# aliabdelkader/FusionTransformer

Measured on AMD Instinct MI355X. Metric: frames/sec fwd+bwd (SemanticKITTI synth), whole job, higher is better.
Workload: dtype f32

## Files before the change

fusiontransformer_amd/_lib.py:

```python
from __future__ import annotations

import ctypes as C
import os

import torch

_HERE = os.path.dirname(os.path.abspath(__file__))
LIB_PATH = os.path.join(_HERE, "csrc", "libftx.so")

_i32, _i64, _f32, _vp, _sz = C.c_int32, C.c_int64, C.c_float, C.c_void_p, C.c_size_t

SIGNATURES = {
    "ftx_version": (C.c_int, []),
    "ftx_last_error": (C.c_char_p, []),
    "ftx_stream_scratch_bytes": (_sz, []),
    "ftx_stream_scratch_attach": (C.c_int, [_vp, _vp, _sz]),
    "ftx_stream_scratch_reset": (C.c_int, [_vp]),
    "ftx_stream_scratch_release": (C.c_int, [_vp]),
    "ftx_hash": (C.c_int, [_vp, _i64, _vp, _vp]),
    "ftx_hash_kernel": (C.c_int, [_vp, _i64, _vp, _i32, _vp, _vp]),
    "ftx_floor_coords": (C.c_int, [_vp, _i64, _i32, _vp, _vp]),
    "ftx_hashtable_capacity": (_i64, [_i64]),
    "ftx_hashtable_build": (C.c_int, [_vp, _i64, _vp, _vp, _i64, _vp]),
    "ftx_hashtable_query": (C.c_int, [_vp, _i64, _vp, _vp, _i64, _vp, _vp]),
    "ftx_count": (C.c_int, [_vp, _i64, _vp, _i64, _vp]),
    "ftx_unique_workspace_bytes": (_sz, [_i64]),
    "ftx_unique_sorted": (C.c_int, [_vp, _i64, _vp, _vp, _vp, _vp, _sz, _vp]),
    "ftx_rotate_points": (C.c_int, [_vp, _i64, _vp, _vp, _vp]),
    "ftx_sorted_rank": (C.c_int, [_vp, _vp, _i64, _vp, _i64, _vp, _vp]),
    "ftx_downsample_coords": (C.c_int, [_vp, _i64, _i32, _vp, _vp]),
    "ftx_gather_coords": (C.c_int, [_vp, _vp, _i64, _vp, _vp]),
    "ftx_levels_workspace_bytes": (_sz, [_i64, _i32]),
    "ftx_levels_unique": (C.c_int, [_vp, _i64, _vp, _i32, _vp, _vp, _vp, _vp, _vp, _vp, _sz, _vp]),
    "ftx_level_segments": (C.c_int, [_vp, _i64, _vp, _i64, _i32, _vp, _vp]),
    "ftx_level_coords": (C.c_int, [_vp, _vp, _i64, _i32, _vp, _vp]),
    "ftx_kernel_map_build": (C.c_int, [_vp, _i64, _vp, _i32, _vp, _vp, _i64, _vp, _vp]),
    "ftx_kernel_map_count_workspace_bytes": (_sz, [_i64, _i32]),
    "ftx_kernel_map_count": (C.c_int, [_vp, _i64, _i32, _vp, _vp, _vp, _sz, _vp]),
    "ftx_kernel_map_pairs": (C.c_int, [_vp, _i64, _i64, _i32, _vp, _vp, _vp, _vp, _i64, _vp]),
    "ftx_trilinear_weights": (C.c_int, [_vp, _vp, _i64, _i32, _vp, _vp]),
    "ftx_voxelize_fwd": (C.c_int, [_vp, _vp, _vp, _i64, _i32, _i64, _vp, _vp]),
    "ftx_voxelize_bwd": (C.c_int, [_vp, _vp, _vp, _i64, _i32, _i64, _vp, _vp]),
    "ftx_devoxelize_fwd": (C.c_int, [_vp, _vp, _vp, _i64, _i32, _i64, _vp, _vp]),
    "ftx_devoxelize_bwd": (C.c_int, [_vp, _vp, _vp, _i64, _i32, _i64, _vp, _vp]),
    "ftx_segment_workspace_bytes": (_sz, [_i64, _i64]),
    "ftx_segment_build": (C.c_int, [_vp, _i64, _i64, _vp, _vp, _vp, _sz, _vp]),
    "ftx_voxelize_fwd_sorted": (C.c_int, [_vp, _vp, _vp, _i64, _i32, _i64, _vp, _vp]),
    "ftx_devoxelize_bwd_sorted": (C.c_int, [_vp, _vp, _vp, _vp, _i64, _i32, _i64, _vp, _vp]),
    "ftx_segment_sum": (C.c_int, [_vp, _vp, _vp, _i64, _i32, _i64, _vp, _vp]),
    "ftx_lift_cells": (C.c_int, [_vp, _vp, _i64, _i32, _i32, _i32, _i32, _i32, _vp, _vp]),
    "ftx_lift_gather_fwd": (C.c_int, [_vp, _vp, _vp, _i64, _i32, _i32, _i32, _i32, _i32, _i32, _vp, _vp]),
    "ftx_lift_gather_bwd": (C.c_int, [_vp, _vp, _vp, _i64, _i32, _i32, _i32, _i32, _i32, _i32, _vp, _vp]),
    "ftx_resample_nearest_fwd": (C.c_int, [_vp, _i32, _i32, _i32, _i32, _i32, _i32, _vp, _vp]),
    "ftx_resample_nearest_bwd": (C.c_int, [_vp, _i32, _i32, _i32, _i32, _i32, _i32, _vp, _vp]),
    "ftx_sample_down_workspace_bytes": (_sz, []),
    "ftx_sample_down_fwd": (C.c_int, [_vp, _i32, _i32, _i32, _i32, _i32, _vp, _vp, _vp, _vp, _vp, _vp, _f32, _f32, _i32, _vp, _vp, _vp, _sz, _vp]),
    "ftx_sample_down_bwd": (C.c_int, [_vp, _vp, _i32, _i32, _i32, _i32, _i32, _vp, _vp, _vp, _vp, _vp, _vp, _vp, _vp, _vp, _sz, _vp]),
    "ftx_affine_sample_fwd": (C.c_int, [_vp, _vp, _i32, _i32, _i32, _i32, _vp, _i32, _i32, _vp, _vp]),
    "ftx_affine_theta_workspace_bytes": (_sz, [_i32]),
    "ftx_affine_sample_bwd_theta": (C.c_int, [_vp, _vp, _i32, _i32, _i32, _i32, _vp, _vp, _i32, _i32, _vp, _vp, _sz, _vp]),
    "ftx_affine_lift_fwd": (C.c_int, [_vp, _vp, _i32, _i32, _i32, _i32, _vp, _vp, _vp, _i64, _i32, _i32, _vp, _vp]),
    "ftx_affine_lift_cells": (C.c_int, [_vp, _vp, _vp, _i64, _i32, _i32, _i32, _i32, _i32, _vp, _vp]),
    "ftx_affine_lift_bwd": (C.c_int, [_vp, _vp, _i32, _i32, _i32, _i32, _vp, _vp, _vp, _vp, _i64, _i32, _i32, _vp, _vp, _vp, _vp, _vp, _sz, _vp]),
    "ftx_loc_conv_pool_relu_fwd_workspace_bytes": (_sz, [_i32, _i32, _i32, _i32]),
    "ftx_loc_conv_pool_relu_fwd": (C.c_int, [_vp, _vp, _i32, _i32, _i32, _i32, _vp, _vp, _i32, _i32, _vp, _vp, _vp, _vp, _sz, _vp]),
    "ftx_loc_conv_pool_relu_bwd_weight_workspace_bytes": (_sz, [_i32, _i32, _i32, _i32, _i32, _i32]),
    "ftx_loc_conv_pool_relu_bwd_weight": (C.c_int, [_vp, _vp, _i32, _i32, _i32, _i32, _vp, _vp, _vp, _i32, _i32, _vp, _vp, _vp, _sz, _vp]),
    "ftx_loc_conv_pool_relu_bwd_data": (C.c_int, [_vp, _vp, _vp, _vp, _i32, _i32, _i32, _i32, _i32, _i32, _vp, _vp, _vp]),
    "ftx_spconv_pairs_gemm": (C.c_int, [_vp, _i64, _vp, _vp, _i32, _vp, _i64, _i32, _i32, _i32, _vp, _vp]),
    "ftx_spconv_pairs_gemm_scatter": (C.c_int, [_vp, _i64, _vp, _vp, _vp, _i32, _vp, _i64, _i32, _i32, _i32, _vp, _i64, _vp]),
    "ftx_spconv_ostat_supported": (_i32, [_i32, _i32, _i32, _i32]),
    "ftx_spconv_ostat_blocks": (_i32, [_i64]),
    "ftx_spconv_ostat": (C.c_int, [_vp, _i64, _vp, _i64, _vp, _i32, _i32, _i32, _i32, _i32, _vp, _vp, _i32, _vp]),
    "ftx_rows_gemm": (C.c_int, [_vp, _i64, _vp, _i32, _vp, _i32, _i32, _vp, _vp]),
    "ftx_spconv_gemm_block_cols": (_i32, [_i32, _i64, _i32]),
    "ftx_spconv_reduce": (C.c_int, [_vp, _vp, _i64, _i32, _i32, _vp, _vp]),
    "ftx_spconv_reduce_bn_eval": (C.c_int, [_vp, _vp, _i64, _i32, _i32, _vp, _vp, _vp, _vp, _vp, _f32, _i32, _vp, _vp]),
    "ftx_spconv_reduce_stats_blocks": (_i32, [_i64, _i32]),
    "ftx_spconv_reduce_stats": (C.c_int, [_vp, _vp, _i64, _i32, _i32, _vp, _vp, _i32, _vp]),
    "ftx_bn_train_fwd_totals": (C.c_int, [_vp, _vp, _vp, _vp, _vp, _vp, _f32, _f32, _i64, _i32, _i32, _vp, _vp, _vp, _vp, _vp]),
    "ftx_spconv_pairs_wgrad_workspace_bytes": (_sz, [_i64, _i32, _i32, _i32]),
    "ftx_spconv_pairs_wgrad": (C.c_int, [_vp, _i64, _vp, _vp, _i64, _vp, _vp, _i64, _i32, _i32, _i32, _vp, _vp, _sz, _vp]),
    "ftx_spconv_wgrad_resident_blocks": (_i32, [_i32, _i32]),
    "ftx_spconv_wgrad_table_blocks": (_i32, [_i32, _i32, _i32, _i32]),
    "ftx_spconv_pairs_gemm_bf16": (C.c_int, [_vp, _i64, _vp, _vp, _i32, _vp, _i64, _i32, _i32, _i32, _vp, _vp]),
    "ftx_spconv_pairs_gemm_scatter_bf16": (C.c_int, [_vp, _i64, _vp, _vp, _vp, _i32, _vp, _i64, _i32, _i32, _i32, _vp, _i64, _vp]),
    "ftx_rows_gemm_bf16": (C.c_int, [_vp, _i64, _vp, _i32, _vp, _i32, _i32, _vp, _vp]),
    "ftx_spconv_pairs_wgrad_bf16_workspace_bytes": (_sz, [_i64, _i32, _i32, _i32]),
    "ftx_spconv_pairs_wgrad_bf16": (C.c_int, [_vp, _i64, _vp, _vp, _i64, _vp, _vp, _i64, _i32, _i32, _i32, _vp, _vp, _sz, _vp]),
    "ftx_spconv_gemm_bf16_block_cols": (_i32, [_i32, _i64, _i32]),
    "ftx_spconv_wgrad_bf16_table_blocks": (_i32, [_i32, _i32, _i32, _i32]),
    "ftx_bn_workspace_bytes": (_sz, [_i64, _i32]),
    "ftx_bn_train_fwd": (C.c_int, [_vp, _vp, _vp, _vp, _vp, _vp, _f32, _f32, _i64, _i32, _i32, _vp, _vp, _vp, _vp, _sz, _vp]),
    "ftx_bn_eval_fwd": (C.c_int, [_vp, _vp, _vp, _vp, _vp, _vp, _f32, _i64, _i32, _i32, _vp, _vp]),
    "ftx_adam_chunk_elements": (_i32, []),
    "ftx_adam_tensor_bytes": (_i32, []),
    "ftx_adam_step": (C.c_int, [_vp, _vp, _vp, _i32, C.c_double, C.c_double, _f32, _f32, _vp]),
    "ftx_add_layernorm_fwd": (C.c_int, [_vp, _vp, _vp, _vp, _vp, _f32, _i64, _i32, _vp, _vp, _vp, _vp, _vp]),
    "ftx_layernorm_bwd_workspace_bytes": (_sz, [_i64, _i32]),
    "ftx_add_layernorm_bwd": (C.c_int, [_vp, _vp, _vp, _vp, _vp, _vp, _i64, _i32, _i32, _vp, _vp, _vp, _sz, _vp]),
    "ftx_colsum_workspace_bytes": (_sz, [_i64, _i32]),
    "ftx_colsum": (C.c_int, [_vp, _i64, _i32, _vp, _vp, _sz, _vp]),
    "ftx_attn_fwd": (C.c_int, [_vp, _i32, _i32, _i32, _i32, _f32, _vp, _vp, _vp]),
    "ftx_attn_bwd_workspace_bytes": (_sz, [_i32, _i32, _i32]),
    "ftx_attn_bwd": (C.c_int, [_vp, _vp, _vp, _vp, _i32, _i32, _i32, _i32, _f32, _vp, _vp, _sz, _vp]),
    "ftx_attn_fwd_tiled": (C.c_int, [_vp, _i32, _i32, _i32, _i32, _f32, _vp, _vp, _i32, _i32, _vp]),
    "ftx_attn_bwd_tiled": (C.c_int, [_vp, _vp, _vp, _vp, _i32, _i32, _i32, _i32, _f32, _vp, _vp, _sz, _i32, _i32, _vp]),
    "ftx_attn_fwd_bf16": (C.c_int, [_vp, _i32, _i32, _i32, _i32, _f32, _vp, _vp, _i32, _i32, _vp]),
    "ftx_attn_bwd_bf16": (C.c_int, [_vp, _vp, _vp, _vp, _i32, _i32, _i32, _i32, _f32, _vp, _vp, _sz, _i32, _i32, _vp]),
    "ftx_dense_gemm_bf16": (C.c_int, [_vp, _vp, _i32, _vp, _vp, _i64, _i32, _i32, _i32, _vp, _vp, _vp]),
    "ftx_dense_wgrad_bf16_workspace_bytes": (_sz, [_i64, _i32, _i32]),
    "ftx_dense_wgrad_bf16": (C.c_int, [_vp, _vp, _i64, _i32, _i32, _vp, _vp, _sz, _vp]),
    "ftx_dense_bf16_tile": (C.c_int, [_i32, _i64, _i32, _i32, _vp, _vp, _vp]),
    "ftx_dense_gemm_split": (C.c_int, [_vp, _vp, _i32, _vp, _vp, _i64, _i32, _i32, _i32, _vp, _vp, _vp]),
    "ftx_dense_wgrad_split_workspace_bytes": (_sz, [_i64, _i32, _i32]),
    "ftx_dense_wgrad_split": (C.c_int, [_vp, _vp, _i64, _i32, _i32, _vp, _vp, _sz, _vp]),
    "ftx_dense_split_tile": (C.c_int, [_i32, _i64, _i32, _i32, _vp, _vp, _vp]),
    "ftx_fusion_loss_workspace_bytes": (_sz, []),
    "ftx_fusion_loss": (C.c_int, [_vp, _vp, _vp, _vp, _vp, _vp, _f32, _i64, _i32, _i32, _vp, _vp, _vp, _vp, _vp, _vp, _vp, _vp, _sz, _vp]),
    "ftx_fusion_loss_mix": (C.c_int, [_vp, _vp, _vp, _vp, _vp, _vp, _f32, _f32, _i64, _i32, _i32, _vp, _vp, _vp, _vp, _vp, _vp, _vp, _vp, _sz, _vp]),
    "ftx_seg_loss_workspace_bytes": (_sz, []),
    "ftx_seg_loss": (C.c_int, [_vp, _vp, _vp, _i64, _i32, _i32, _vp, _vp, _vp, _vp, _sz, _vp]),
    "ftx_project_points": (C.c_int, [_vp, _i64, _vp, _i32, _i32, _vp, _vp, _vp]),
    "ftx_eval_scatter_back": (C.c_int, [_vp, _vp, _i64, _i32, _vp, _vp, _i64, _vp, _vp, _vp, _vp, _vp, _vp, _vp, _vp, _vp]),
    "ftx_bn_train_bwd": (C.c_int, [_vp, _vp, _vp, _vp, _vp, _vp, _vp, _i64, _i32, _i32, _vp, _vp, _vp, _vp, _vp, _sz, _vp]),
    "ftx_color_jitter_workspace_bytes": (_sz, [_i32, _i32]),
    "ftx_color_jitter_u8": (C.c_int, [_vp, _i64, _i32, _i32, _i32, _vp, _vp, _i32, _vp, _vp, _sz, _vp]),
    "ftx_color_jitter_chw": (C.c_int, [_vp, _i64, _i32, _i32, _i32, _vp, _vp, _i32, _i32, _vp, _vp, _vp, _vp, _sz, _vp]),
    "ftx_resize_ksize": (_i32, [_i32, _i32]),
    "ftx_resize_coeffs_host": (C.c_int, [_i32, _i32, _vp, _vp]),
    "ftx_resize_workspace_bytes": (_sz, [_i32, _i32, _i32, _i32, _i32]),
    "ftx_resize_bilinear_u8": (C.c_int, [_vp, _i64, _i64, _i32, _i32, _i32, _i32, _vp, _vp, _i32, _vp, _vp, _i32, _i32, _i32, _vp, _vp, _sz, _vp]),
    "ftx_rows_concat": (C.c_int, [_vp, _i32, _vp, _i32, _i64, _vp, _vp]),
    "ftx_rows_add": (C.c_int, [_vp, _vp, _i64, _i32, _vp, _vp]),
    "ftx_spvcnn_layer_bytes": (_i32, []),
    "ftx_spvcnn_op_bytes": (_i32, []),
    "ftx_spvcnn_map_bytes": (_i32, []),
    "ftx_spvcnn_pv_bytes": (_i32, []),
    "ftx_spvcnn_eval_arena_bytes": (_sz, [_vp, _i32, _vp, _i32, _vp, _vp, _i32, _vp, _i32, _vp]),
    "ftx_spvcnn_eval": (C.c_int, [_vp, _i32, _vp, _i32, _vp, _vp, _i32, _vp, _i32, _vp, _vp, _i32, _i32, _vp, _vp, _vp, _sz, _vp, _vp]),
    "ftx_rows_split": (C.c_int, [_vp, _i64, _i32, _i32, _vp, _vp, _vp]),
    "ftx_spvcnn_train_layer_bytes": (_i32, []),
    "ftx_spvcnn_train_pv_bytes": (_i32, []),
    "ftx_spvcnn_train_arena_bytes": (_sz, [_vp, _i32, _vp, _i32, _vp, _vp, _i32, _vp, _i32, _vp, _vp]),
    "ftx_spvcnn_train_fwd": (C.c_int, [_vp, _vp, _i32, _vp, _i32, _vp, _vp, _i32, _vp, _i32, _vp, _vp, _i32, _i32, _vp, _vp, _vp, _vp, _sz, _vp, _vp, _vp]),
    "ftx_spvcnn_train_bwd": (C.c_int, [_vp, _vp, _i32, _vp, _i32, _vp, _vp, _i32, _vp, _vp, _i32, _vp, _vp, _i32, _i32, _vp, _vp, _vp, _sz, _vp, _vp]),
    "ftx_spvcnn_index_layout_words": (_i32, []),
    "ftx_spvcnn_index_layout": (C.c_int, [_i64, _i32, _vp, _vp, _i32, _vp]),
    "ftx_spvcnn_index_levels_arena_bytes": (_sz, [_i64]),
    "ftx_spvcnn_index_maps_arena_bytes": (_sz, [_i64, _i32, _vp, _i32]),
    "ftx_spvcnn_index_pairs_arena_bytes": (_sz, [_i64, _vp, _vp]),
    "ftx_spvcnn_index_levels": (C.c_int, [_vp, _i64, _f32, _f32, _vp, _sz, _vp, _vp]),
    "ftx_spvcnn_index_maps": (C.c_int, [_vp, _i64, _f32, _f32, _vp, _i32, _vp, _i32, _vp, _sz, _vp, _sz, _vp, _vp]),
# ... 60 lines not shown
```

fusiontransformer_amd/csrc/ftx_spconv.hip:

```cpp
#include <cstring>
#include <cstdlib>
#include "ftx_bn_eval_op.h"
#include "ftx_index_ops.h"
#include "ftx_spconv_common.h"
#include <rocprim/device/device_scan.hpp>
#include <rocprim/iterator/transform_iterator.hpp>

using namespace ftx;

struct IsValid {
  __host__ __device__ int32_t operator()(int32_t v) const { return v >= 0 ? 1 : 0; }
};

extern "C" size_t ftx_kernel_map_count_workspace_bytes(int64_t n_out, int32_t k) {
  if (n_out <= 0 || k <= 0) return 256;
  size_t bytes = 0;
  const int32_t *in = nullptr;
  int32_t *out = nullptr;
  auto it = rocprim::make_transform_iterator(in, IsValid());
  if (rocprim::exclusive_scan(nullptr, bytes, it, out, 0, (size_t)(n_out * k), rocprim::plus<int32_t>()) != hipSuccess) return 0;
  return bytes + 256;
}

__global__ void koff_kernel(const int32_t *__restrict__ nbr, const int32_t *__restrict__ scan, int64_t n_out, int k, int32_t *__restrict__ koff) {
  int t = blockIdx.x * blockDim.x + threadIdx.x;
  if (t <= k) koff[t] = koff_entry(nbr, scan, n_out, k, t, 0);
}

extern "C" int ftx_kernel_map_count(const int32_t *nbr, int64_t n_out, int32_t k, int32_t *pos, int32_t *koff, void *workspace,
                                    size_t workspace_bytes, void *stream) {
  FTX_REQUIRE(n_out >= 0 && k >= 1, "ftx_kernel_map_count: bad size");
  FTX_REQUIRE(koff, "ftx_kernel_map_count: null koff");
  hipStream_t st = (hipStream_t)stream;
  if (n_out == 0) {
    if (hipMemsetAsync(koff, 0, sizeof(int32_t) * (k + 1), st) != hipSuccess) return check_launch("ftx_kernel_map_count memset");
    return FTX_OK;
  }
  FTX_REQUIRE(nbr && pos && workspace, "ftx_kernel_map_count: null pointer");
  FTX_REQUIRE(n_out * k < 0x7fffffff, "ftx_kernel_map_count: map too large for int32 positions");
  size_t need = ftx_kernel_map_count_workspace_bytes(n_out, k);
  if (workspace_bytes < need) return workspace_short("ftx_kernel_map_count", workspace_bytes, need);
  size_t bytes = workspace_bytes;
  auto it = rocprim::make_transform_iterator(nbr, IsValid());
  if (rocprim::exclusive_scan(workspace, bytes, it, pos, 0, (size_t)(n_out * k), rocprim::plus<int32_t>(), st) != hipSuccess) {
    set_error("ftx_kernel_map_count: scan failed");
    return FTX_ELAUNCH;
  }
  koff_kernel<<<1, 64, 0, st>>>(nbr, pos, n_out, k, koff);
  return check_launch("ftx_kernel_map_count");
}

__global__ void fill_m1_kernel(int32_t *__restrict__ p, int64_t n) {
  for (int64_t i = blockIdx.x * (int64_t)blockDim.x + threadIdx.x; i < n; i += (int64_t)gridDim.x * blockDim.x) p[i] = -1;
}

__global__ void pairs_scatter_kernel(const int32_t *__restrict__ nbr, int64_t n_out, int64_t n_in, int k, int32_t *__restrict__ pos,
                                     int32_t *__restrict__ pos_t, int32_t *__restrict__ pair_in, int32_t *__restrict__ pair_out,
                                     int64_t cap) {
  const int64_t total = n_out * k;
  for (int64_t e = blockIdx.x * (int64_t)blockDim.x + threadIdx.x; e < total; e += (int64_t)gridDim.x * blockDim.x) {
    if (pair_entry(nbr[e], pos[e], e, n_out, n_in, cap, pair_in, pair_out, pos_t) < 0) pos[e] = -1;
  }
}

extern "C" int ftx_kernel_map_pairs(const int32_t *nbr, int64_t n_out, int64_t n_in, int32_t k, int32_t *pos, int32_t *pos_t, int32_t *pair_in,
                                    int32_t *pair_out, int64_t n_pairs, void *stream) {
  FTX_REQUIRE(n_out >= 0 && n_in >= 0 && k >= 1 && n_pairs >= 0, "ftx_kernel_map_pairs: bad size");
  hipStream_t st = (hipStream_t)stream;
  if (n_in > 0) {
    FTX_REQUIRE(pos_t, "ftx_kernel_map_pairs: null pos_t");
    fill_m1_kernel<<<grid_for(n_in * k, 256), 256, 0, st>>>(pos_t, n_in * k);
  }
  if (n_out == 0) return check_launch("ftx_kernel_map_pairs");
  FTX_REQUIRE(nbr && pos && (n_pairs == 0 || (pair_in && pair_out)), "ftx_kernel_map_pairs: null pointer");
  pairs_scatter_kernel<<<grid_for(n_out * k, 256), 256, 0, st>>>(nbr, n_out, n_in, k, pos, pos_t, pair_in, pair_out, n_pairs);
  return check_launch("ftx_kernel_map_pairs");
}

constexpr int AS_STRIDE = 36;

template <int NT>
__global__ __launch_bounds__(256) void pairs_gemm_kernel(const float *__restrict__ A, int64_t rows_a, const int32_t *__restrict__ gather,
                                                         const float *__restrict__ W, int w_transposed, const int32_t *__restrict__ koff,
                                                         int ca, int co, int kvol, float *__restrict__ tmp, const float *__restrict__ bias,
                                                         int64_t n_dense, const int32_t *__restrict__ scatter, int64_t rows_out) {
  constexpr int BN = 32 * NT;
  constexpr int BS_STRIDE = AS_STRIDE;
  constexpr int A_PASSES = kPairAPasses;
  constexpr int B_PASSES = NT;

  __shared__ __attribute__((aligned(16))) float As[kPairTile * AS_STRIDE];
  __shared__ __attribute__((aligned(16))) float Bs[BN * BS_STRIDE];
  __shared__ int s_tile[3];

  const int tid = threadIdx.x;
  gemm_tile_scan(koff, kvol, n_dense, gather == nullptr, s_tile);
  __syncthreads();
  const int k = s_tile[0];
  if (k < 0) return;
  const int p0 = s_tile[1], cnt = s_tile[2];

  const int wave = tid >> 6, lane = tid & 63;
  const int half = lane >> 5, l31 = lane & 31;
  const int n0 = blockIdx.y * BN;
  const int arow = tid >> 3, acol = (tid & 7) * 4;

  const bool kfull = (ca % kPairBK) == 0;
  int32_t src[A_PASSES];
  pair_gather_rows(gather, p0, cnt, rows_a, src);
  const float *Wk = W + (int64_t)k * ca * co;

  f32x16 acc[NT];
#pragma unroll
  for (int j = 0; j < NT; ++j)
#pragma unroll
    for (int g = 0; g < 16; ++g) acc[j][g] = 0.f;

  float4 ra[A_PASSES], rb[B_PASSES];
  auto load_chunk = [&](int c0) {
    if (kfull) {
#pragma unroll
      for (int p = 0; p < A_PASSES; ++p) ra[p] = *(const float4 *)&A[(int64_t)src[p] * ca + c0 + acol];
#pragma unroll
      for (int q = 0; q < B_PASSES; ++q) {
        if (!w_transposed) {
          int kk = ((tid >> 6) << 3) + (tid & 7), n4 = n0 + (q * 8 + ((tid >> 3) & 7)) * 4;
          n4 = n4 + 4 <= co ? n4 : co - 4;
          rb[q] = *(const float4 *)&Wk[(int64_t)(c0 + kk) * co + n4];
        } else {
          int e = q * 256 + tid;
          int nn = n0 + (e >> 3), k4 = (e & 7) * 4;
          nn = nn < co ? nn : co - 1;
          rb[q] = *(const float4 *)&Wk[(int64_t)nn * ca + c0 + k4];
        }
      }
      return;
    }
#pragma unroll
    for (int p = 0; p < A_PASSES; ++p) {
      float4 v = make_float4(0.f, 0.f, 0.f, 0.f);
      if (c0 + acol < ca) v = *(const float4 *)&A[(int64_t)src[p] * ca + c0 + acol];
      ra[p] = v;
    }
#pragma unroll
    for (int q = 0; q < B_PASSES; ++q) {
      float4 v = make_float4(0.f, 0.f, 0.f, 0.f);
      if (!w_transposed) {
        int kk = ((tid >> 6) << 3) + (tid & 7), n4 = (q * 8 + ((tid >> 3) & 7)) * 4;
        if (c0 + kk < ca && n0 + n4 < co) v = *(const float4 *)&Wk[(int64_t)(c0 + kk) * co + n0 + n4];
      } else {
        int e = q * 256 + tid;
        int nn = e >> 3, k4 = (e & 7) * 4;
        if (n0 + nn < co && c0 + k4 < ca) v = *(const float4 *)&Wk[(int64_t)(n0 + nn) * ca + c0 + k4];
      }
      rb[q] = v;
    }
  };
  auto store_chunk = [&]() {
#pragma unroll
    for (int p = 0; p < A_PASSES; ++p) *(float4 *)&As[(p * 32 + arow) * AS_STRIDE + acol] = ra[p];
#pragma unroll
    for (int q = 0; q < B_PASSES; ++q) {
      if (!w_transposed) {
        int kk = ((tid >> 6) << 3) + (tid & 7), n4 = (q * 8 + ((tid >> 3) & 7)) * 4;
        Bs[(n4 + 0) * BS_STRIDE + kk] = rb[q].x;
        Bs[(n4 + 1) * BS_STRIDE + kk] = rb[q].y;
        Bs[(n4 + 2) * BS_STRIDE + kk] = rb[q].z;
        Bs[(n4 + 3) * BS_STRIDE + kk] = rb[q].w;
      } else {
        int e = q * 256 + tid;
        int nn = e >> 3, k4 = (e & 7) * 4;
        *(float4 *)&Bs[nn * BS_STRIDE + k4] = rb[q];
      }
    }
  };

  load_chunk(0);
  for (int c0 = 0; c0 < ca; c0 += kPairBK) {
    store_chunk();
    __syncthreads();
    if (c0 + kPairBK < ca) load_chunk(c0 + kPairBK);
    const float *arow_p = &As[(wave * 32 + l31) * AS_STRIDE + 4 * half];
    const float *brow_p = &Bs[l31 * BS_STRIDE + 4 * half];
    float af[2][4], bf[2][NT][4];
    auto load_frag = [&](int buf, int t) {
      float4 a = *(const float4 *)(arow_p + 8 * t);
      af[buf][0] = a.x; af[buf][1] = a.y; af[buf][2] = a.z; af[buf][3] = a.w;
#pragma unroll
      for (int j = 0; j < NT; ++j) {
        float4 b = *(const float4 *)(brow_p + j * 32 * BS_STRIDE + 8 * t);
        bf[buf][j][0] = b.x; bf[buf][j][1] = b.y; bf[buf][j][2] = b.z; bf[buf][j][3] = b.w;
      }
    };
    load_frag(0, 0);
#pragma unroll
    for (int t = 0; t < kPairBK / 8; ++t) {
      if (t + 1 < kPairBK / 8) load_frag((t + 1) & 1, t + 1);
#pragma unroll
      for (int s = 0; s < 4; ++s)
#pragma unroll
        for (int j = 0; j < NT; ++j) acc[j] = __builtin_amdgcn_mfma_f32_32x32x2f32(bf[t & 1][j][s], af[t & 1][s], acc[j], 0, 0, 0);
    }
    __syncthreads();
  }
  pair_gemm_epilogue<NT>(acc, p0, cnt, n0, gather, rows_a, scatter, rows_out, bias, co, tmp);
}

#include "ftx_lastblock.h"


template <int KVOL>
__device__ __forceinline__ float4 reduce_row(const float *__restrict__ tmp, const int32_t *__restrict__ pos, int64_t n, int co, int kvol,
                                             int64_t r, int j) {
  float4 acc = make_float4(0.f, 0.f, 0.f, 0.f);
  if (KVOL > 0) {
    int32_t p[KVOL > 0 ? KVOL : 1];
#pragma unroll
    for (int k = 0; k < KVOL; ++k) p[k] = pos[(int64_t)k * n + r];
#pragma unroll
    for (int k = 0; k < KVOL; ++k) {
      if (p[k] >= 0) {
        float4 v = *(const float4 *)&tmp[(int64_t)p[k] * co + j];
        acc.x += v.x; acc.y += v.y; acc.z += v.z; acc.w += v.w;
      }
    }
  } else {
    for (int k = 0; k < kvol; ++k) {
      int32_t q = pos[(int64_t)k * n + r];
      if (q >= 0) {
        float4 v = *(const float4 *)&tmp[(int64_t)q * co + j];
        acc.x += v.x; acc.y += v.y; acc.z += v.z; acc.w += v.w;
      }
    }
  }
  return acc;
}

template <int KVOL>
__global__ void spconv_reduce_kernel(const float *__restrict__ tmp, const int32_t *__restrict__ pos, int64_t n, int co, int kvol,
                                     float *__restrict__ out) {
  const int cv = co >> 2;
  const int64_t total = n * cv;
  for (int64_t e = blockIdx.x * (int64_t)blockDim.x + threadIdx.x; e < total; e += (int64_t)gridDim.x * blockDim.x) {
    int64_t r = e / cv;
    int j = (int)(e - r * cv) * 4;
    const float4 acc = reduce_row<KVOL>(tmp, pos, n, co, kvol, r, j);
    *(float4 *)&out[r * co + j] = acc;
  }
}

static unsigned reduce_grid(int64_t n, int co) {
  int64_t g = ceil_div(n * (co / 4), 256);
  if (g > 8192) g = 8192;
  return (unsigned)g;
}

extern "C" int ftx_spconv_reduce(const float *tmp, const int32_t *pos, int64_t n, int32_t co, int32_t kvol, float *out, void *stream) {
  FTX_REQUIRE(n >= 0 && kvol >= 1 && co >= 4 && co % 4 == 0, "ftx_spconv_reduce: bad size");
  if (n == 0) return FTX_OK;
  FTX_REQUIRE(pos && out, "ftx_spconv_reduce: null pointer");
  const unsigned g = reduce_grid(n, co);
  hipStream_t st = (hipStream_t)stream;
  if (kvol == 27)
    spconv_reduce_kernel<27><<<g, 256, 0, st>>>(tmp, pos, n, co, kvol, out);
  else if (kvol == 8)
    spconv_reduce_kernel<8><<<g, 256, 0, st>>>(tmp, pos, n, co, kvol, out);
  else
    spconv_reduce_kernel<0><<<g, 256, 0, st>>>(tmp, pos, n, co, kvol, out);
  return check_launch("ftx_spconv_reduce");
}

template <int KVOL>
__global__ void spconv_reduce_bn_eval_kernel(const float *__restrict__ tmp, const int32_t *__restrict__ pos, int64_t n, int co,
                                             const float *__restrict__ res, const float *__restrict__ gamma, const float *__restrict__ beta,
                                             const float *__restrict__ rm, const float *__restrict__ rv, float eps, int relu,
                                             float *__restrict__ out) {
  const int cv = co >> 2;
  const int64_t total = n * cv;
  for (int64_t e = blockIdx.x * (int64_t)blockDim.x + threadIdx.x; e < total; e += (int64_t)gridDim.x * blockDim.x) {
    int64_t r = e / cv;
    int j = (int)(e - r * cv) * 4;
    const float4 acc = reduce_row<KVOL>(tmp, pos, n, co, KVOL, r, j);
    *(float4 *)&out[r * co + j] = bn_eval_apply4(acc, res, r * co + j, rm, rv, eps, gamma, beta, j, relu);
  }
}

extern "C" int ftx_spconv_reduce_bn_eval(const float *tmp, const int32_t *pos, int64_t n, int32_t co, int32_t kvol, const float *residual,
                                         const float *gamma, const float *beta, const float *running_mean, const float *running_var,
// ... 149 lines not shown
        if (p >= rend || s_ok[(p - rbase) & (kWgradRound - 1)] == 0) rg[q] = make_float4(0.f, 0.f, 0.f, 0.f);
      }
    }
#pragma unroll
    for (int q = 0; q < QA; ++q) *(float4 *)&As[(q * 256 + tid) * 4] = ra[q];
#pragma unroll
    for (int q = 0; q < QG; ++q) *(float4 *)&Gs[(q * 256 + tid) * 4] = rg[q];
  };
  const float *ap = As + wm * 32 * MI + MI * l31, *gp = Gs + wn * 32 * NI + NI * l31;
  auto mfma_step = [&]() {
    constexpr int ITS = WG_BR / 2 / KS;
    float af[2][MI], gf[2][NI];
    auto frag = [&](int buf, int it) {
      const int kk = 2 * (it * KS + ks) + half;
      FragLoad<MI>::ld(ap + kk * TM, af[buf]);
      FragLoad<NI>::ld(gp + kk * TN, gf[buf]);
    };
    frag(0, 0);
#pragma unroll
    for (int it = 0; it < ITS; ++it) {
      if (it + 1 < ITS) frag((it + 1) & 1, it + 1);
#pragma unroll
      for (int i = 0; i < MI; ++i)
#pragma unroll
        for (int j = 0; j < NI; ++j)
          acc[i][j] = __builtin_amdgcn_mfma_f32_32x32x2f32(gf[it & 1][j], af[it & 1][i], acc[i][j], 0, 0, 0);
    }
  };

  for (rbase = lo; rbase < hi; rbase += kWgradRound) {
    rend = (rbase + kWgradRound < hi) ? rbase + kWgradRound : hi;
    wgrad_stage_indices(idx_a, rows_a, idx_g, rows_g, rbase, rend, s_ia, s_ig, s_ok, &s_bad);
    load_step(rbase, ra0, rg0);
    load_step(rbase + WG_BR, ra1, rg1);
    for (int p0 = rbase; p0 < rend; p0 += 2 * WG_BR) {
      store_step(p0, ra0, rg0);
      __syncthreads();
      load_step(p0 + 2 * WG_BR, ra0, rg0);
      mfma_step();
      __syncthreads();
      if (p0 + WG_BR >= rend) break;
      store_step(p0 + WG_BR, ra1, rg1);
      __syncthreads();
      load_step(p0 + 3 * WG_BR, ra1, rg1);
      mfma_step();
      __syncthreads();
    }
  }

  wgrad_ks_reduce<MI, NI, KS>(acc, lds, wq, ks, lane);

  if (ks == 0) {
    const int64_t mat = (int64_t)ca * cg;
    float *dst = single ? dW + (int64_t)k * mat : part + (int64_t)blockIdx.x * mat;
    const int ab = m0 + wm * 32 * MI + MI * l31, gb = n0 + wn * 32 * NI;
#pragma unroll
    for (int i = 0; i < MI; ++i) {
      const int row = ab + i;
      if (row < ca) {
#pragma unroll
        for (int q = 0; q < 4; ++q) {
          float v[4 * NI];
#pragma unroll
          for (int e = 0; e < 4; ++e)
#pragma unroll
            for (int j = 0; j < NI; ++j) v[e * NI + j] = acc[i][j][4 * q + e];
          const int col = gb + NI * (8 * q + 4 * half);
#pragma unroll
          for (int t = 0; t < NI; ++t)
            if (col + 4 * t < cg) *(float4 *)&dst[(int64_t)row * cg + col + 4 * t] = make_float4(v[4 * t], v[4 * t + 1], v[4 * t + 2], v[4 * t + 3]);
        }
      }
    }
  }
}

struct SpconvF32 {
  static constexpr const char *pairs_name = "ftx_spconv_pairs_gemm", *scatter_name = "ftx_spconv_pairs_gemm_scatter", *rows_name = "ftx_rows_gemm",
                              *wgrad_name = "ftx_spconv_pairs_wgrad";
  static constexpr int wgrad_blocks[4][4] = {{8, 4, 3, 3}, {5, 3, 2, 2}, {4, 2, 1, 2}, {3, 2, 2, 2}};
  static constexpr int wgrad_step = 2 * WG_BR;
  template <int NT>
  static void gemm(dim3 grid, hipStream_t st, const PairsGemmArgs &a) {
    pairs_gemm_kernel<NT><<<grid, 256, 0, st>>>(a.A, a.rows_a, a.gather, a.W, a.w_transposed, a.koff, a.ca, a.co, a.kvol, a.out, a.bias, a.n_dense,
                                                a.scatter, a.rows_out);
  }
  template <int MI, int NI, int WMG, int WNG>
  static void wgrad(dim3 grid, hipStream_t st, const PairsWgradArgs &a) {
    pairs_wgrad_kernel<MI, NI, WMG, WNG><<<grid, 256, 0, st>>>(a.A, a.rows_a, a.idx_a, a.G, a.rows_g, a.idx_g, a.koff, a.ca, a.cg, a.kvol, a.tile_len,
                                                               a.part, a.dW, a.n_dense);
  }
};

extern "C" int32_t ftx_spconv_gemm_block_cols(int32_t co, int64_t n_pairs, int32_t kvol) { return spconv_gemm_block_cols(co, n_pairs, kvol); }

extern "C" int ftx_spconv_pairs_gemm(const float *A, int64_t rows_a, const int32_t *gather, const float *W, int32_t w_transposed,
                                     const int32_t *koff, int64_t n_pairs, int32_t ca, int32_t co, int32_t kvol, float *tmp, void *stream) {
  return spconv_pairs_entry<SpconvF32>(false, A, rows_a, gather, nullptr, W, w_transposed, koff, n_pairs, ca, co, kvol, tmp, 0, stream);
}

extern "C" int ftx_spconv_pairs_gemm_scatter(const float *A, int64_t rows_a, const int32_t *gather, const int32_t *scatter, const float *W,
                                             int32_t w_transposed, const int32_t *koff, int64_t n_pairs, int32_t ca, int32_t co, int32_t kvol,
                                             float *out, int64_t rows_out, void *stream) {
  return spconv_pairs_entry<SpconvF32>(true, A, rows_a, gather, scatter, W, w_transposed, koff, n_pairs, ca, co, kvol, out, rows_out, stream);
}

extern "C" int ftx_rows_gemm(const float *A, int64_t n, const float *W, int32_t w_transposed, const float *bias, int32_t ca, int32_t co,
                             float *out, void *stream) {
  return spconv_rows_entry<SpconvF32>(A, n, W, w_transposed, bias, ca, co, out, stream);
}

extern "C" int32_t ftx_spconv_wgrad_table_blocks(int32_t mi, int32_t wmg, int32_t ni, int32_t wng) {
  return spconv_wgrad_table_blocks<SpconvF32>(mi, wmg, ni, wng);
}
extern "C" int32_t ftx_spconv_wgrad_resident_blocks(int32_t ca, int32_t cg) { return spconv_wgrad_occ<SpconvF32>(spconv_wgrad_config(ca, cg)); }

extern "C" size_t ftx_spconv_pairs_wgrad_workspace_bytes(int64_t n_pairs, int32_t ca, int32_t cg, int32_t kvol) {
  return spconv_wgrad_workspace_bytes<SpconvF32>(n_pairs, ca, cg, kvol);
}

extern "C" int ftx_spconv_pairs_wgrad(const float *A, int64_t rows_a, const int32_t *idx_a, const float *G, int64_t rows_g, const int32_t *idx_g,
                                      const int32_t *koff, int64_t n_pairs, int32_t ca, int32_t cg, int32_t kvol, float *dW, void *workspace,
                                      size_t workspace_bytes, void *stream) {
  return spconv_wgrad_entry<SpconvF32>(A, rows_a, idx_a, G, rows_g, idx_g, koff, n_pairs, ca, cg, kvol, dW, workspace, workspace_bytes, stream);
}
```

fusiontransformer_amd/csrc/ftx_spconv_bf16.hip:

```cpp
#include "ftx_spconv_common.h"

using namespace ftx;

__device__ inline bf16x4 round4(float4 v) { return (bf16x4){(__bf16)v.x, (__bf16)v.y, (__bf16)v.z, (__bf16)v.w}; }

constexpr int GB_STRIDE = 40;

template <int NT>
__global__ __launch_bounds__(256) void pairs_gemm_bf16_kernel(const float *__restrict__ A, int64_t rows_a, const int32_t *__restrict__ gather,
                                                              const float *__restrict__ W, int w_transposed, const int32_t *__restrict__ koff,
                                                              int ca, int co, int kvol, float *__restrict__ tmp, const float *__restrict__ bias,
                                                              int64_t n_dense, const int32_t *__restrict__ scatter, int64_t rows_out) {
  constexpr int BN = 32 * NT;
  constexpr int A_PASSES = kPairAPasses;
  constexpr int B_PASSES = NT;
  __shared__ __attribute__((aligned(16))) __bf16 As[kPairTile * GB_STRIDE];
  __shared__ __attribute__((aligned(16))) __bf16 Bs[BN * GB_STRIDE];
  __shared__ int s_tile[3];

  const int tid = threadIdx.x;
  gemm_tile_scan(koff, kvol, n_dense, gather == nullptr, s_tile);
  __syncthreads();
  const int k = s_tile[0];
  if (k < 0) return;
// ... 188 lines not shown
      for (int e = 0; e < 4; ++e) *(bf16x2 *)&At[(ra_row[q] + e) * WB_STRIDE + pa[q]] = (bf16x2){x0[e], x1[e]};
    }
#pragma unroll
    for (int q = 0; q < QG; ++q) {
      const bf16x4 x0 = round4(rg[q][0]), x1 = round4(rg[q][1]);
#pragma unroll
      for (int e = 0; e < 4; ++e) *(bf16x2 *)&Gt[(rg_row[q] + e) * WB_STRIDE + pg[q]] = (bf16x2){x0[e], x1[e]};
    }
  };
  const __bf16 *ap = At + (wm * MI * 32 + l31) * WB_STRIDE + 8 * half;
  const __bf16 *gp = Gt + (wn * NI * 32 + l31) * WB_STRIDE + 8 * half;
  auto mfma_step = [&]() {
#pragma unroll
    for (int it = 0; it < 4 / KS; ++it) {
      const int s = it * KS + ks;
      bf16x8 af[MI], gf[NI];
#pragma unroll
      for (int i = 0; i < MI; ++i) af[i] = *(const bf16x8 *)(ap + i * 32 * WB_STRIDE + 16 * s);
#pragma unroll
      for (int j = 0; j < NI; ++j) gf[j] = *(const bf16x8 *)(gp + j * 32 * WB_STRIDE + 16 * s);
#pragma unroll
      for (int i = 0; i < MI; ++i)
#pragma unroll
        for (int j = 0; j < NI; ++j) acc[i][j] = mfma_bf16(gf[j], af[i], acc[i][j]);
    }
  };

  for (rbase = lo; rbase < hi; rbase += kWgradRound) {
    rend = (rbase + kWgradRound < hi) ? rbase + kWgradRound : hi;
    wgrad_stage_indices(idx_a, rows_a, idx_g, rows_g, rbase, rend, s_ia, s_ig, s_ok, &s_bad);
    load_step(rbase);
    for (int p0 = rbase; p0 < rend; p0 += WB_BR) {
      store_step(p0);
      __syncthreads();
      if (p0 + WB_BR < rend) load_step(p0 + WB_BR);
      mfma_step();
      __syncthreads();
    }
  }

  wgrad_ks_reduce<MI, NI, KS>(acc, (float *)lds, wq, ks, lane);

  if (ks == 0) {
    const int64_t mat = (int64_t)ca * cg;
    float *dst = single ? dW + (int64_t)k * mat : part + (int64_t)blockIdx.x * mat;
#pragma unroll
    for (int i = 0; i < MI; ++i) {
      const int row = m0 + (wm * MI + i) * 32 + l31;
      if (row < ca) {
#pragma unroll
        for (int j = 0; j < NI; ++j)
#pragma unroll
          for (int q = 0; q < 4; ++q) {
            const int col = n0 + (wn * NI + j) * 32 + 8 * q + 4 * half;
            if (col < cg)
              *(float4 *)&dst[(int64_t)row * cg + col] = make_float4(acc[i][j][4 * q], acc[i][j][4 * q + 1], acc[i][j][4 * q + 2], acc[i][j][4 * q + 3]);
          }
      }
    }
  }
}

struct SpconvBf16 {
  static constexpr const char *pairs_name = "ftx_spconv_pairs_gemm_bf16", *scatter_name = "ftx_spconv_pairs_gemm_scatter_bf16",
                              *rows_name = "ftx_rows_gemm_bf16", *wgrad_name = "ftx_spconv_pairs_wgrad_bf16";
  static constexpr int wgrad_blocks[4][4] = {{8, 4, 3, 3}, {4, 3, 2, 2}, {3, 2, 1, 2}, {3, 2, 2, 2}};
  static constexpr int wgrad_step = 2 * WB_BR;
  template <int NT>
  static void gemm(dim3 grid, hipStream_t st, const PairsGemmArgs &a) {
    pairs_gemm_bf16_kernel<NT><<<grid, 256, 0, st>>>(a.A, a.rows_a, a.gather, a.W, a.w_transposed, a.koff, a.ca, a.co, a.kvol, a.out, a.bias, a.n_dense,
                                                     a.scatter, a.rows_out);
  }
  template <int MI, int NI, int WMG, int WNG>
  static void wgrad(dim3 grid, hipStream_t st, const PairsWgradArgs &a) {
    pairs_wgrad_bf16_kernel<MI, NI, WMG, WNG><<<grid, 256, 0, st>>>(a.A, a.rows_a, a.idx_a, a.G, a.rows_g, a.idx_g, a.koff, a.ca, a.cg, a.kvol,
                                                                    a.tile_len, a.part, a.dW, a.n_dense);
  }
};

extern "C" int32_t ftx_spconv_gemm_bf16_block_cols(int32_t co, int64_t n_pairs, int32_t kvol) { return spconv_gemm_block_cols(co, n_pairs, kvol); }

extern "C" int ftx_spconv_pairs_gemm_bf16(const float *A, int64_t rows_a, const int32_t *gather, const float *W, int32_t w_transposed,
                                          const int32_t *koff, int64_t n_pairs, int32_t ca, int32_t co, int32_t kvol, float *tmp, void *stream) {
  return spconv_pairs_entry<SpconvBf16>(false, A, rows_a, gather, nullptr, W, w_transposed, koff, n_pairs, ca, co, kvol, tmp, 0, stream);
}

extern "C" int ftx_spconv_pairs_gemm_scatter_bf16(const float *A, int64_t rows_a, const int32_t *gather, const int32_t *scatter, const float *W,
                                                  int32_t w_transposed, const int32_t *koff, int64_t n_pairs, int32_t ca, int32_t co, int32_t kvol,
                                                  float *out, int64_t rows_out, void *stream) {
  return spconv_pairs_entry<SpconvBf16>(true, A, rows_a, gather, scatter, W, w_transposed, koff, n_pairs, ca, co, kvol, out, rows_out, stream);
}

extern "C" int ftx_rows_gemm_bf16(const float *A, int64_t n, const float *W, int32_t w_transposed, const float *bias, int32_t ca, int32_t co,
                                  float *out, void *stream) {
  return spconv_rows_entry<SpconvBf16>(A, n, W, w_transposed, bias, ca, co, out, stream);
}

extern "C" int32_t ftx_spconv_wgrad_bf16_table_blocks(int32_t mi, int32_t wmg, int32_t ni, int32_t wng) {
  return spconv_wgrad_table_blocks<SpconvBf16>(mi, wmg, ni, wng);
}

extern "C" size_t ftx_spconv_pairs_wgrad_bf16_workspace_bytes(int64_t n_pairs, int32_t ca, int32_t cg, int32_t kvol) {
  return spconv_wgrad_workspace_bytes<SpconvBf16>(n_pairs, ca, cg, kvol);
}

extern "C" int ftx_spconv_pairs_wgrad_bf16(const float *A, int64_t rows_a, const int32_t *idx_a, const float *G, int64_t rows_g, const int32_t *idx_g,
                                           const int32_t *koff, int64_t n_pairs, int32_t ca, int32_t cg, int32_t kvol, float *dW, void *workspace,
                                           size_t workspace_bytes, void *stream) {
  return spconv_wgrad_entry<SpconvBf16>(A, rows_a, idx_a, G, rows_g, idx_g, koff, n_pairs, ca, cg, kvol, dW, workspace, workspace_bytes, stream);
}
```

fusiontransformer_amd/csrc/ftx_spconv_common.h:

```cpp
#pragma once
#include "ftx_common.h"
#include "ftx_mfma.h"

namespace ftx {

constexpr int kPairTile = 128;
constexpr int kPairBK = 32;
constexpr int kPairAPasses = 4;
constexpr int kWgradRound = 1024;
constexpr int kWgradCUs = 256;

template <bool RANGE>
__device__ __forceinline__ void pair_tile_scan(const int32_t *__restrict__ koff, int kvol, int tile, int n_dense, int *s_tile) {
  const int tid = threadIdx.x, b = blockIdx.x;
  if (tid >= 64) return;
  int c = 0;
  if (tid < kvol) c = koff ? koff[tid + 1] - koff[tid] : n_dense;
  int nt = (c + tile - 1) / tile;
  int incl = nt;
#pragma unroll
  for (int off = 1; off < 64; off <<= 1) {
    int v = __shfl_up(incl, off, 64);
    if (tid >= off) incl += v;
  }
  int excl = incl - nt;
  bool mine = (tid < kvol) && b >= excl && b < incl;
  unsigned long long m = __ballot(mine);
  if (mine) {
    int t = b - excl;
    int left = c - t * tile;
    int first = (koff ? koff[tid] : 0) + t * tile;
    s_tile[0] = tid;
    s_tile[1] = first;
    s_tile[2] = (RANGE ? first : 0) + (left > tile ? tile : left);
    if (RANGE) s_tile[3] = nt;
  }
  if (m == 0ull && tid == 0) s_tile[0] = -1;
}

__device__ __forceinline__ void gemm_tile_scan(const int32_t *__restrict__ koff, int kvol, int64_t n_dense, bool dense, int *s_tile) {
  if (!dense) {
    __builtin_assume(koff != nullptr);
    return pair_tile_scan<false>(koff, kvol, kPairTile, 0, s_tile);
  }
  if (threadIdx.x == 0) {
    int64_t left = n_dense - (int64_t)blockIdx.x * kPairTile;
    s_tile[0] = left > 0 ? 0 : -1;
    s_tile[1] = blockIdx.x * kPairTile;
    s_tile[2] = left > kPairTile ? kPairTile : (int)left;
  }
}

__device__ __forceinline__ void pair_gather_rows(const int32_t *__restrict__ gather, int p0, int cnt, int64_t rows_a, int32_t (&src)[kPairAPasses]) {
  const int arow = threadIdx.x >> 3;
#pragma unroll
  for (int p = 0; p < kPairAPasses; ++p) {
    int r = p * 32 + arow;
    int32_t s = 0;
    if (r < cnt) s = gather ? gather[p0 + r] : p0 + r;
    if (s < 0 || s >= rows_a) s = 0;
    src[p] = s;
  }
}

template <int NT>
__device__ __forceinline__ void pair_gemm_epilogue(const f32x16 (&acc)[NT], int p0, int cnt, int n0, const int32_t *__restrict__ gather, int64_t rows_a,
                                          const int32_t *__restrict__ scatter, int64_t rows_out, const float *__restrict__ bias, int co,
                                          float *__restrict__ out) {
  const int wave = threadIdx.x >> 6, lane = threadIdx.x & 63;
  const int half = lane >> 5, l31 = lane & 31;
  const bool nfull = n0 + 32 * NT <= co;
  const int row = wave * 32 + l31;
  int64_t drow = row < cnt ? p0 + row : -1;
  bool zero = false;
  if (gather != nullptr && drow >= 0) {
    const int32_t sidx = gather[drow];
    zero = sidx < 0 || sidx >= rows_a;
  }
  if (scatter != nullptr && drow >= 0) {
    drow = scatter[drow];
    if (drow >= rows_out) drow = -1;
  }
  if (drow < 0) return;
  float *dst = out + drow * co;
#pragma unroll
  for (int j = 0; j < NT; ++j)
#pragma unroll
    for (int q = 0; q < 4; ++q) {
      const int col = n0 + j * 32 + 8 * q + 4 * half;
      if (nfull || col < co) {
        float4 v = make_float4(acc[j][4 * q], acc[j][4 * q + 1], acc[j][4 * q + 2], acc[j][4 * q + 3]);
        if (zero) v = make_float4(0.f, 0.f, 0.f, 0.f);
        if (bias) {
          const float4 bv = *(const float4 *)&bias[col];
          v.x += bv.x; v.y += bv.y; v.z += bv.z; v.w += bv.w;
        }
        *(float4 *)&dst[col] = v;
      }
    }
}

__device__ __forceinline__ void wgrad_stage_indices(const int32_t *__restrict__ idx_a, int64_t rows_a, const int32_t *__restrict__ idx_g, int64_t rows_g,
                                           int rbase, int rend, int32_t *s_ia, int32_t *s_ig, uint8_t *s_ok, int *s_bad) {
  __syncthreads();
  if (threadIdx.x == 0) *s_bad = 0;
  __syncthreads();
  for (int t = threadIdx.x; t < kWgradRound; t += 256) {
    int32_t ia = 0, ig = 0;
    uint8_t ok = 0;
    if (t < rend - rbase) {
      ia = idx_a ? idx_a[rbase + t] : rbase + t;
      ig = idx_g ? idx_g[rbase + t] : rbase + t;
      ok = 1;
      if (ia < 0 || ia >= rows_a || ig < 0 || ig >= rows_g) {
        ia = ig = 0;
        ok = 0;
        *s_bad = 1;
      }
    }
    s_ia[t] = ia;
    s_ig[t] = ig;
    s_ok[t] = ok;
  }
  __syncthreads();
}

template <int MI, int NI, int KS>
__device__ __forceinline__ void wgrad_ks_reduce(f32x16 (&acc)[MI][NI], float *red, int wq, int ks, int lane) {
  for (int r = 1; r < KS; ++r) {
    if (ks == r) {
#pragma unroll
      for (int i = 0; i < MI; ++i)
#pragma unroll
        for (int j = 0; j < NI; ++j) {
          const f32x16 v = acc[i][j];
#pragma unroll
          for (int g = 0; g < 16; ++g) red[(((wq * MI + i) * NI + j) * 16 + g) * 64 + lane] = v[g];
        }
    }
    __syncthreads();
    if (ks == 0) {
#pragma unroll
      for (int i = 0; i < MI; ++i)
#pragma unroll
        for (int j = 0; j < NI; ++j) {
          f32x16 v = acc[i][j];
#pragma unroll
          for (int g = 0; g < 16; ++g) v[g] += red[(((wq * MI + i) * NI + j) * 16 + g) * 64 + lane];
          acc[i][j] = v;
        }
    }
    __syncthreads();
  }
}

}

template <int TL>
__global__ __launch_bounds__(256) void wgrad_reduce_kernel(const float *__restrict__ part, const int32_t *__restrict__ koff, int kvol,
                                                           int tile_len, int n_dense, int64_t mat, float *__restrict__ dW) {
  constexpr int COLS = 256 / TL;
  __shared__ float4 sh[TL][COLS];
  const int k = blockIdx.y;
  int first = 0, cnt = 0;
  for (int q = 0; q <= k; ++q) {
    int c = koff ? koff[q + 1] - koff[q] : n_dense;
    int nt = (c + tile_len - 1) / tile_len;
    if (q < k) first += nt; else cnt = nt;
  }
  if (cnt == 1) return;
  const int col = threadIdx.x % COLS, tl = threadIdx.x / COLS;
  const int64_t chunks = ftx::ceil_div(mat / 4, COLS);
  for (int64_t chunk = blockIdx.x; chunk < chunks; chunk += gridDim.x) {
    const int64_t e = (chunk * COLS + col) * 4;
    float4 s = make_float4(0.f, 0.f, 0.f, 0.f);
    if (e < mat) {
      const float *src = part + (int64_t)first * mat + e;
      int t = tl;
      for (; t + 3 * TL < cnt; t += 4 * TL) {
        float4 v0 = *(const float4 *)&src[(int64_t)t * mat], v1 = *(const float4 *)&src[(int64_t)(t + TL) * mat];
        float4 v2 = *(const float4 *)&src[(int64_t)(t + 2 * TL) * mat], v3 = *(const float4 *)&src[(int64_t)(t + 3 * TL) * mat];
        s.x += v0.x; s.y += v0.y; s.z += v0.z; s.w += v0.w;
        s.x += v1.x; s.y += v1.y; s.z += v1.z; s.w += v1.w;
        s.x += v2.x; s.y += v2.y; s.z += v2.z; s.w += v2.w;
        s.x += v3.x; s.y += v3.y; s.z += v3.z; s.w += v3.w;
      }
      for (; t < cnt; t += TL) {
        float4 v = *(const float4 *)&src[(int64_t)t * mat];
        s.x += v.x; s.y += v.y; s.z += v.z; s.w += v.w;
      }
    }
    if (TL > 1) {
      sh[tl][col] = s;
      __syncthreads();
      if (tl == 0) {
#pragma unroll
        for (int l = 1; l < TL; ++l) {
          float4 v = sh[l][col];
          s.x += v.x; s.y += v.y; s.z += v.z; s.w += v.w;
        }
      }
      __syncthreads();
    }
    if (tl == 0 && e < mat) *(float4 *)&dW[(int64_t)k * mat + e] = s;
  }
}

namespace ftx {

inline void launch_wgrad_reduce(const float *part, const int32_t *koff, int kvol, int tile_len, int n_dense, int64_t mat, int64_t tiles, float *dW,
                                hipStream_t st) {
  const int64_t big_tiles = kvol > 1 ? 6 * tiles / kvol : tiles;
  const int64_t want_blocks = ceil_div(1024, kvol);
  auto rgrid = [&](int cols) { int64_t c = ceil_div(mat / 4, cols); return dim3((unsigned)(c < want_blocks ? c : want_blocks), (unsigned)kvol); };
  if (big_tiles <= 4)
    wgrad_reduce_kernel<1><<<rgrid(256), 256, 0, st>>>(part, koff, kvol, tile_len, n_dense, mat, dW);
  else if (big_tiles <= 32)
    wgrad_reduce_kernel<4><<<rgrid(64), 256, 0, st>>>(part, koff, kvol, tile_len, n_dense, mat, dW);
  else
    wgrad_reduce_kernel<16><<<rgrid(16), 256, 0, st>>>(part, koff, kvol, tile_len, n_dense, mat, dW);
}

struct PairsGemmArgs {
  const float *A;
  int64_t rows_a;
  const int32_t *gather;
  const float *W;
  int w_transposed;
  const int32_t *koff;
  int ca, co, kvol;
  float *out;
  const float *bias;
  int64_t n_dense;
  const int32_t *scatter;
  int64_t rows_out;
};

inline int spconv_gemm_nt(int co, int64_t row_tiles) {
  int nt = co >= 128 ? 4 : (co + 31) / 32;
  if (co > 128 && co % 96 == 0 && co % 128 != 0) nt = 3;
  if (nt == 4 && row_tiles * ceil_div(co, 128) <= 400) nt = 2;
  return nt;
}

inline int32_t spconv_gemm_block_cols(int32_t co, int64_t n_pairs, int32_t kvol) {
  if (co < 4 || co % 4 != 0 || n_pairs < 0 || kvol < 0) return -1;
  return 32 * spconv_gemm_nt(co, ceil_div(n_pairs, kPairTile) + kvol);
}

template <class F>
void spconv_launch_gemm(int64_t row_tiles, hipStream_t st, const PairsGemmArgs &a) {
  const int nt = spconv_gemm_nt(a.co, row_tiles);
  const dim3 grid((unsigned)row_tiles, (unsigned)ceil_div(a.co, 32 * nt));
  switch (nt) {
    case 1: F::template gemm<1>(grid, st, a); break;
    case 2: F::template gemm<2>(grid, st, a); break;
    case 3: F::template gemm<3>(grid, st, a); break;
    default: F::template gemm<4>(grid, st, a); break;
  }
}

template <class F>
int spconv_pairs_entry(bool scattered, const float *A, int64_t rows_a, const int32_t *gather, const int32_t *scatter, const float *W,
                       int32_t w_transposed, const int32_t *koff, int64_t n_pairs, int32_t ca, int32_t co, int32_t kvol, float *out, int64_t rows_out,
                       void *stream) {
  const char *me = scattered ? F::scatter_name : F::pairs_name;
  FTX_REQUIRE(n_pairs >= 0 && rows_a >= 0 && rows_out >= 0 && kvol >= 1 && kvol <= 64, "%s: bad size", me);
  FTX_REQUIRE(ca >= 4 && ca % 4 == 0 && co >= 4 && co % 4 == 0, "%s: channels must be multiples of 4 (ca=%d co=%d)", me, ca, co);
  if (n_pairs == 0) return FTX_OK;
  FTX_REQUIRE(A && gather && (scatter || !scattered) && W && koff && out && rows_a >= 1, "%s: null pointer or empty operand", me);
  const PairsGemmArgs a = {A, rows_a, gather, W, w_transposed, koff, ca, co, kvol, out, nullptr, 0, scatter, rows_out};
  spconv_launch_gemm<F>(ceil_div(n_pairs, kPairTile) + kvol, (hipStream_t)stream, a);
  return check_launch(me);
}

template <class F>
int spconv_rows_entry(const float *A, int64_t n, const float *W, int32_t w_transposed, const float *bias, int32_t ca, int32_t co, float *out,
                      void *stream) {
  const char *me = F::rows_name;
  FTX_REQUIRE(n >= 0, "%s: n < 0", me);
  FTX_REQUIRE(ca >= 4 && ca % 4 == 0 && co >= 4 && co % 4 == 0, "%s: channels must be multiples of 4 (ca=%d co=%d)", me, ca, co);
  if (n == 0) return FTX_OK;
  FTX_REQUIRE(A && W && out, "%s: null pointer", me);
  const PairsGemmArgs a = {A, n, nullptr, W, w_transposed, nullptr, ca, co, 1, out, bias, n, nullptr, 0};
  spconv_launch_gemm<F>(ceil_div(n, kPairTile), (hipStream_t)stream, a);
  return check_launch(me);
}

struct PairsWgradArgs {
  const float *A;
  int64_t rows_a;
  const int32_t *idx_a;
  const float *G;
  int64_t rows_g;
  const int32_t *idx_g, *koff;
  int ca, cg, kvol, tile_len;
  float *part, *dW;
  int n_dense;
};

struct WgradCfg { int mi, wmg, ni, wng; };
inline WgradCfg spconv_wgrad_config(int ca, int cg) {
  WgradCfg c;
  if (ca <= 32) { c.mi = 1; c.wmg = 1; }
  else if (ca <= 64) { c.mi = 2; c.wmg = 1; }
  else if (ca % 96 == 0 && ca % 128 != 0) { c.mi = 3; c.wmg = 1; }
  else { c.mi = 2; c.wmg = 2; }
  if (cg <= 32) { c.ni = 1; c.wng = 1; }
  else if (cg <= 64) { c.ni = 2; c.wng = 1; }
  else if (cg % 96 == 0 && cg % 128 != 0) { c.ni = 3; c.wng = 1; }
  else { c.ni = 2; c.wng = 2; }
  if (c.mi == 3 && c.ni == 3) { c.mi = 2; c.wmg = 2; }
  return c;
}

template <class F>
int spconv_wgrad_occ(const WgradCfg &c) {
  auto side = [](int i, int w) { return w == 2 ? 3 : i - 1; };
  return F::wgrad_blocks[side(c.mi, c.wmg)][side(c.ni, c.wng)];
}
template <class F>
int32_t spconv_wgrad_table_blocks(int32_t mi, int32_t wmg, int32_t ni, int32_t wng) {
  if (!((mi >= 1 && mi <= 3 && wmg == 1) || (mi == 2 && wmg == 2)) || !((ni >= 1 && ni <= 3 && wng == 1) || (ni == 2 && wng == 2))) return -1;
  return spconv_wgrad_occ<F>(WgradCfg{mi, wmg, ni, wng});
}

template <class F>
int spconv_wgrad_tile_len(int64_t n_pairs, int ca, int cg, int kvol) {
  const WgradCfg c = spconv_wgrad_config(ca, cg);
  const int64_t mn_tiles = ceil_div(ca, 32 * c.mi * c.wmg) * ceil_div(cg, 32 * c.ni * c.wng);
  const int64_t slots = (int64_t)kWgradCUs * spconv_wgrad_occ<F>(c);
  int64_t len = 256;
  for (int rounds = 1; rounds <= 64; ++rounds) {
    int64_t tiles = (slots * rounds * 15 / 16) / mn_tiles - (kvol + 1) / 2;
    if (tiles < 1) tiles = 1;
    len = ceil_div(ceil_div(n_pairs, tiles), F::wgrad_step) * F::wgrad_step;
    if (len <= 4096) break;
  }
  if (len < 256) len = 256;
  return (int)len;
}

inline int64_t spconv_wgrad_tiles_ub(int64_t n_pairs, int tile_len, int kvol) { return ceil_div(n_pairs, tile_len) + kvol; }

template <class F>
size_t spconv_wgrad_workspace_bytes(int64_t n_pairs, int32_t ca, int32_t cg, int32_t kvol) {
  if (n_pairs <= 0 || ca <= 0 || cg <= 0 || kvol <= 0) return 256;
  const int len = spconv_wgrad_tile_len<F>(n_pairs, ca, cg, kvol);
  return sizeof(float) * (size_t)spconv_wgrad_tiles_ub(n_pairs, len, kvol) * ca * cg;
}

template <class F, int MI, int WMG>
void spconv_launch_wgrad_n(const WgradCfg &c, dim3 grid, hipStream_t st, const PairsWgradArgs &a) {
  if (c.ni == 1) F::template wgrad<MI, 1, WMG, 1>(grid, st, a);
  else if (c.ni == 3) F::template wgrad<MI, 3, WMG, 1>(grid, st, a);
  else if (c.wng == 1) F::template wgrad<MI, 2, WMG, 1>(grid, st, a);
  else F::template wgrad<MI, 2, WMG, 2>(grid, st, a);
}

template <class F>
int spconv_wgrad_entry(const float *A, int64_t rows_a, const int32_t *idx_a, const float *G, int64_t rows_g, const int32_t *idx_g,
                       const int32_t *koff, int64_t n_pairs, int32_t ca, int32_t cg, int32_t kvol, float *dW, void *workspace,
                       size_t workspace_bytes, void *stream) {
  const char *me = F::wgrad_name;
  FTX_REQUIRE(n_pairs >= 0 && rows_a >= 0 && rows_g >= 0 && kvol >= 1 && kvol <= 64, "%s: bad size", me);
  FTX_REQUIRE(ca >= 4 && ca % 4 == 0 && cg >= 4 && cg % 4 == 0, "%s: channels must be multiples of 4 (ca=%d cg=%d)", me, ca, cg);
  FTX_REQUIRE(dW, "%s: null dW", me);
// ... 32 lines not shown
```

fusiontransformer_amd/functional.py:

```python
from __future__ import annotations

import ctypes
import functools

import numpy as np
import torch

from . import _lib
from ._lib import check, ptr, req, stream

I32, I64, F32 = torch.int32, torch.int64, torch.float32


def _empty(shape, dtype, like):
    return torch.empty(shape, dtype=dtype, device=like.device)


_SCRATCH = {}
_WS_BYTES = {}


def _ws_bytes(fn_name, *args):
    key = (fn_name,) + args
    v = _WS_BYTES.get(key)
# ... 168 lines not shown


def sorted_rank(sorted_keys: torch.Tensor, n_sorted: torch.Tensor, queries: torch.Tensor) -> torch.Tensor:
    L = _lib.load()
    req(sorted_keys, I64, "sorted_rank sorted", 1)
    req(n_sorted, I32, "sorted_rank n_sorted", 1)
    req(queries, I64, "sorted_rank queries", 1)
    rank = _empty((queries.shape[0],), I32, queries)
    check(L.ftx_sorted_rank(ptr(sorted_keys), ptr(n_sorted), sorted_keys.shape[0], ptr(queries), queries.shape[0], ptr(rank), stream()), "ftx_sorted_rank")
    return rank


def rotate_points(points: torch.Tensor, rot) -> torch.Tensor:
    L = _lib.load()
    req(points, F32, "rotate_points points", 2)
    if points.shape[1] != 3:
        raise ValueError("rotate_points: points must be (N, 3)")
    r = np.ascontiguousarray(np.asarray(rot, dtype=np.float32).reshape(9))
    out = _empty(tuple(points.shape), F32, points)
    check(L.ftx_rotate_points(ptr(points), points.shape[0], r.ctypes.data_as(ctypes.c_void_p), ptr(out), stream()), "ftx_rotate_points")
    return out


def downsample_coords(coords: torch.Tensor, ratio: int) -> torch.Tensor:
    L = _lib.load()
    req(coords, I32, "downsample coords", 2)
    out = torch.empty_like(coords)
    check(L.ftx_downsample_coords(ptr(coords), coords.shape[0], int(ratio), ptr(out), stream()), "ftx_downsample_coords")
    return out


def gather_coords(src: torch.Tensor, index: torch.Tensor) -> torch.Tensor:
    L = _lib.load()
    req(src, I32, "gather_coords src", 2)
    req(index, I32, "gather_coords index", 1)
    out = _empty((index.shape[0], 4), I32, src)
    check(L.ftx_gather_coords(ptr(src), ptr(index), index.shape[0], ptr(out), stream()), "ftx_gather_coords")
    return out


def kernel_offsets(kernel_size: int, tensor_stride: int = 1) -> np.ndarray:
    single = (np.arange(-kernel_size // 2 + 1, kernel_size // 2 + 1) * tensor_stride).tolist()
    if kernel_size % 2 == 1:
        offs = [[x, y, z] for z in single for y in single for x in single]
    else:
        offs = [[x, y, z] for x in single for y in single for z in single]
    return np.array(offs, dtype=np.int32)


def kernel_map_build(out_coords: torch.Tensor, offsets: torch.Tensor, table: HashTable) -> torch.Tensor:
    L = _lib.load()
    req(out_coords, I32, "kernel_map out_coords", 2)
    req(offsets, I32, "kernel_map offsets", 2)
    n_out, k = out_coords.shape[0], offsets.shape[0]
    nbr = _empty((k, n_out), I32, out_coords)
    check(L.ftx_kernel_map_build(ptr(out_coords), n_out, ptr(offsets), k, ptr(table.keys), ptr(table.vals), table.capacity, ptr(nbr), stream()),
          "ftx_kernel_map_build")
    return nbr


def kernel_map_count(nbr: torch.Tensor):
    L = _lib.load()
    req(nbr, I32, "kernel_map_count nbr", 2)
    k, n_out = nbr.shape
    pos = torch.empty_like(nbr)
    koff = _empty((k + 1,), I32, nbr)
    ws_bytes = _ws_bytes("ftx_kernel_map_count_workspace_bytes", n_out, k)
    ws = _scratch(ws_bytes, nbr)
    check(L.ftx_kernel_map_count(ptr(nbr), n_out, k, ptr(pos), ptr(koff), ptr(ws), ws_bytes, stream()), "ftx_kernel_map_count")
    return pos, koff


def kernel_map_pairs(nbr: torch.Tensor, pos: torch.Tensor, n_in: int, n_pairs: int):
    L = _lib.load()
    k, n_out = nbr.shape
    pos_t = _empty((k, int(n_in)), I32, nbr)
    pair_in = _empty((int(n_pairs),), I32, nbr)
    pair_out = _empty((int(n_pairs),), I32, nbr)
    check(L.ftx_kernel_map_pairs(ptr(nbr), n_out, int(n_in), k, ptr(pos), ptr(pos_t), ptr(pair_in), ptr(pair_out), int(n_pairs), stream()),
          "ftx_kernel_map_pairs")
    return pos, pos_t, pair_in, pair_out


def calc_ti_weights(pc: torch.Tensor, idx_query: torch.Tensor, scale: int = 1) -> torch.Tensor:
    L = _lib.load()
    req(pc, F32, "calc_ti_weights pc", 2)
    req(idx_query, I32, "calc_ti_weights idx", 2)
    n = pc.shape[0]
    if pc.shape[1] != 4 or idx_query.shape != (n, 8):
        raise ValueError("calc_ti_weights: pc must be (N,4) and idx (N,8)")
    w = _empty((n, 8), F32, pc)
    check(L.ftx_trilinear_weights(ptr(pc), ptr(idx_query), n, int(scale), ptr(w), stream()), "ftx_trilinear_weights")
    return w


class Segments:
    __slots__ = ("order", "seg_off", "m")

    @classmethod
    def from_parts(cls, order, seg_off, m):
        self = cls.__new__(cls)
        self.order, self.seg_off, self.m = order, seg_off, int(m)
        return self

    def __init__(self, keys: torch.Tensor, m: int):
        L = _lib.load()
        keys = req(keys.contiguous().view(-1), I32, "segment keys", 1)
        n = keys.shape[0]
        self.m = int(m)
        self.order = _empty((n,), I32, keys)
        self.seg_off = _empty((self.m + 1,), I32, keys)
        ws_bytes = _ws_bytes("ftx_segment_workspace_bytes", n, self.m)
        ws = _scratch(ws_bytes, keys)
        check(L.ftx_segment_build(ptr(keys), n, self.m, ptr(self.order), ptr(self.seg_off), ptr(ws), ws_bytes, stream()), "ftx_segment_build")


def voxelize_segments(idx: torch.Tensor, m: int) -> Segments:
    return Segments(idx, m)


def devoxelize_segments(idx: torch.Tensor, weights: torch.Tensor, m: int) -> Segments:
    keys = torch.where(weights != 0, idx, torch.full_like(idx, -1))
    return Segments(keys, m)


class _Voxelize(torch.autograd.Function):
    @staticmethod
    def forward(ctx, feats, idx, counts, seg):
        L = _lib.load()
        feats = req(feats.contiguous(), F32, "spvoxelize feats", 2)
        req(idx, I32, "spvoxelize idx", 1)
        req(counts, I32, "spvoxelize counts", 1)
        n, c = feats.shape
        if idx.shape[0] != n:
            raise ValueError("spvoxelize: idx length != rows of feats")
        m = counts.shape[0]
        out = _empty((m, c), F32, feats)
        if seg is not None and c % 4 == 0:
            if seg.m != m or seg.order.shape[0] != n:
                raise ValueError("spvoxelize: segments do not match idx / counts")
            check(L.ftx_voxelize_fwd_sorted(ptr(feats), ptr(seg.order), ptr(seg.seg_off), n, c, m, ptr(out), stream()), "ftx_voxelize_fwd_sorted")
        else:
            check(L.ftx_voxelize_fwd(ptr(feats), ptr(idx), ptr(counts), n, c, m, ptr(out), stream()), "ftx_voxelize_fwd")
        ctx.save_for_backward(idx, counts)
        ctx.n = n
        return out

    @staticmethod
    def backward(ctx, grad_out):
        L = _lib.load()
        idx, counts = ctx.saved_tensors
        grad_out = req(grad_out.contiguous(), F32, "spvoxelize grad", 2)
        m, c = grad_out.shape
        gf = _empty((ctx.n, c), F32, grad_out)
        check(L.ftx_voxelize_bwd(ptr(grad_out), ptr(idx), ptr(counts), ctx.n, c, m, ptr(gf), stream()), "ftx_voxelize_bwd")
        return gf, None, None, None


def spvoxelize(feats, idx, counts, seg=None):
    return _Voxelize.apply(feats, idx, counts, seg)


class _Devoxelize(torch.autograd.Function):
    @staticmethod
    def forward(ctx, feats, idx, weights, seg):
        L = _lib.load()
        feats = req(feats.contiguous(), F32, "spdevoxelize feats", 2)
        req(idx, I32, "spdevoxelize idx", 2)
        req(weights, F32, "spdevoxelize weights", 2)
        m, c = feats.shape
        n = idx.shape[0]
        if idx.shape != (n, 8) or weights.shape != (n, 8):
            raise ValueError("spdevoxelize: idx and weights must be (N,8)")
        out = _empty((n, c), F32, feats)
        check(L.ftx_devoxelize_fwd(ptr(feats), ptr(idx), ptr(weights), n, c, m, ptr(out), stream()), "ftx_devoxelize_fwd")
        ctx.save_for_backward(idx, weights)
        ctx.m, ctx.seg = m, seg
        return out

    @staticmethod
    def backward(ctx, grad_out):
        L = _lib.load()
        idx, weights = ctx.saved_tensors
        grad_out = req(grad_out.contiguous(), F32, "spdevoxelize grad", 2)
        n, c = grad_out.shape
        gf = _empty((ctx.m, c), F32, grad_out)
        seg = ctx.seg
        if seg is not None:
            if seg.m != ctx.m or seg.order.shape[0] != n * 8:
                raise ValueError("spdevoxelize: segments do not match idx")
            check(L.ftx_devoxelize_bwd_sorted(ptr(grad_out), ptr(weights), ptr(seg.order), ptr(seg.seg_off), n, c, ctx.m, ptr(gf), stream()),
                  "ftx_devoxelize_bwd_sorted")
        else:
            check(L.ftx_devoxelize_bwd(ptr(grad_out), ptr(idx), ptr(weights), n, c, ctx.m, ptr(gf), stream()), "ftx_devoxelize_bwd")
        return gf, None, None, None


def spdevoxelize(feats, idx, weights, seg=None):
    _refuse_grad(weights, "spdevoxelize", "weights", "they are computed from the point coordinates, detach them")
    return _Devoxelize.apply(feats, idx, weights, seg)


LAUNCH_LOG = None


def _log_launch(kind, meta, launch):
    if LAUNCH_LOG is None:
        return launch()
    e0, e1 = torch.cuda.Event(enable_timing=True), torch.cuda.Event(enable_timing=True)
    e0.record()
    out = launch()
    e1.record()
    LAUNCH_LOG.append((kind, e0, e1, meta))
    return out


_PAIRS_GEMM = {False: ("ftx_spconv_pairs_gemm", "spconv_pairs_gemm"), True: ("ftx_spconv_pairs_gemm_bf16", "spconv_pairs_gemm_bf16")}
_PAIRS_GEMM_SCATTER = {False: "ftx_spconv_pairs_gemm_scatter", True: "ftx_spconv_pairs_gemm_scatter_bf16"}
_PAIRS_WGRAD = {False: ("ftx_spconv_pairs_wgrad", "ftx_spconv_pairs_wgrad_workspace_bytes", "spconv_pairs_wgrad"),
                True: ("ftx_spconv_pairs_wgrad_bf16", "ftx_spconv_pairs_wgrad_bf16_workspace_bytes", "spconv_pairs_wgrad_bf16")}
_ROWS_GEMM = {False: "ftx_rows_gemm", True: "ftx_rows_gemm_bf16"}


def _launch_pairs(a, rows_a, gather, w, w_transposed, pos, koff, n_pairs, ca, co, kvol, tmp, out, n_out, st, bf16, part=0, nb=0):
    L = _lib.load()
    gemm, kind = _PAIRS_GEMM[bf16]
    meta = dict(pairs=n_pairs, n_out=n_out, ca=ca, co=co, kvol=kvol)
    _log_launch(kind, meta, lambda: check(getattr(L, gemm)(a, rows_a, gather, w, w_transposed, koff, n_pairs, ca, co, kvol, tmp, st), gemm))
    if part:
        _log_launch("spconv_reduce", meta, lambda: check(L.ftx_spconv_reduce_stats(tmp, pos, n_out, co, kvol, out, part, nb, st), "ftx_spconv_reduce_stats"))
    else:
        _log_launch("spconv_reduce", meta, lambda: check(L.ftx_spconv_reduce(tmp, pos, n_out, co, kvol, out, st), "ftx_spconv_reduce"))


def _launch_direct(a, rows_a, gather, scatter, w, w_transposed, koff, n_pairs, ca, co, kvol, out, n_out, st, bf16):
    L = _lib.load()
    gemm = _PAIRS_GEMM_SCATTER[bf16]
    _log_launch(_PAIRS_GEMM[bf16][1], dict(pairs=n_pairs, n_out=n_out, ca=ca, co=co, kvol=kvol, direct=True), lambda: check(getattr(L, gemm)(
        a, rows_a, gather, scatter, w, w_transposed, koff, n_pairs, ca, co, kvol, out, n_out, st), gemm))


def _launch_ostat(a, rows_a, nbr, n_out, w, w_transposed, flip, ca, co, kvol, out, part, nb, st, pairs):
    L = _lib.load()
    _log_launch("spconv_ostat", dict(pairs=pairs, n_out=n_out, ca=ca, co=co, kvol=kvol, direct=True), lambda: check(L.ftx_spconv_ostat(
        a, rows_a, nbr, n_out, w, w_transposed, flip, ca, co, kvol, out, part, nb, st), "ftx_spconv_ostat"))


def _launch_wgrad(a, rows_a, idx_a, g, rows_g, idx_g, koff, n_pairs, ca, cg, kvol, dw, ws, ws_bytes, st, bf16):
    L = _lib.load()
    fn, _, kind = _PAIRS_WGRAD[bf16]
    _log_launch(kind, dict(pairs=n_pairs, n_out=rows_g, ca=ca, co=cg, kvol=kvol), lambda: check(getattr(L, fn)(
        a, rows_a, idx_a, g, rows_g, idx_g, koff, n_pairs, ca, cg, kvol, dw, ws, ws_bytes, st), fn))


def _launch_bn_fwd(x, residual, gamma, beta, running_mean, running_var, momentum, eps, n, c, relu, y, mean, invstd, st, ws=0, ws_bytes=0, totals=0):
    L = _lib.load()
    args = (x, residual, gamma, beta, running_mean, running_var, float(momentum), float(eps), n, c, int(relu), y, mean, invstd)
    if totals:
        _log_launch("bn_fwd", dict(n=n, c=c, reads=1 + (residual != 0), writes=1), lambda: check(L.ftx_bn_train_fwd_totals(*args, totals, st), "ftx_bn_train_fwd_totals"))
    else:
        _log_launch("bn_fwd", dict(n=n, c=c, reads=2 + (residual != 0), writes=1), lambda: check(L.ftx_bn_train_fwd(*args, ws, ws_bytes, st), "ftx_bn_train_fwd"))


def _launch_bn_bwd(gy, x, y, gamma, beta, mean, invstd, n, c, relu, gx, gres, ggamma, gbeta, ws, ws_bytes, st):
    L = _lib.load()
    has_res = gres != 0
    _log_launch("bn_bwd", dict(n=n, c=c, reads=2 * (2 + (1 if (relu and has_res) else 0)), writes=1 + (1 if has_res else 0)), lambda: check(
        L.ftx_bn_train_bwd(gy, x, y, gamma, beta, mean, invstd, n, c, int(relu), gx, gres, ggamma, gbeta, ws, ws_bytes, st), "ftx_bn_train_bwd"))


def _spconv_apply(A, W, gather, pos, koff, n_pairs, n_rows_out, co, w_transposed, bf16=False):
    rows_a, ca = A.shape
    tmp = _empty((n_pairs, co), F32, A)
    out = _empty((n_rows_out, co), F32, A)
    _launch_pairs(ptr(A), rows_a, ptr(gather), ptr(W), int(w_transposed), ptr(pos), ptr(koff), n_pairs, ca, co, koff.shape[0] - 1, ptr(tmp), ptr(out),
                  n_rows_out, stream(), bool(bf16))
    return out


def _spconv_direct(A, W, gather, scatter, koff, n_pairs, n_rows_out, co, w_transposed, bf16=False):
    rows_a, ca = A.shape
    if n_pairs != n_rows_out:
        raise ValueError("direct sparse conv: the pair list must cover every destination row exactly once")
    out = _empty((n_rows_out, co), F32, A)
    _launch_direct(ptr(A), rows_a, ptr(gather), ptr(scatter), ptr(W), int(w_transposed), ptr(koff), n_pairs, ca, co, koff.shape[0] - 1, ptr(out),
                   n_rows_out, stream(), bool(bf16))
    return out


_OSTAT_OK = {}
_OSTAT_MAX_ROWS = 64 * 4096


def ostat_supported(ca, co, kvol, w_transposed=False, rows=0):
    key = (int(ca), int(co), int(kvol), bool(w_transposed))
    v = _OSTAT_OK.get(key)
    if v is None:
        v = _OSTAT_OK[key] = bool(_lib.load().ftx_spconv_ostat_supported(key[0], key[1], key[2], int(key[3])))
    return v and rows <= _OSTAT_MAX_ROWS


def ostat_preferred(ca, co, kvol, w_transposed=False, rows=0):
    return ostat_supported(ca, co, kvol, w_transposed, rows) and not w_transposed and co == 32 and ca <= 32


def _spconv_ostat(A, W, nbr, n_rows_out, co, w_transposed, flip, part=0, nb=0, pairs=0):
    rows_a, ca = A.shape
    kvol = nbr.shape[0]
    if nbr.shape[1] != n_rows_out:
        raise ValueError("ostat sparse conv: the neighbour table does not match the output rows")
    out = _empty((n_rows_out, co), F32, A)
    _launch_ostat(ptr(A), rows_a, ptr(nbr), n_rows_out, ptr(W), int(w_transposed), int(flip), ca, co, kvol, ptr(out), part, nb,
                  _stream_scratch() if part else stream(), pairs)
    return out


def _spconv_wgrad(A, idx_a, G, idx_g, koff, n_pairs, bf16=False):
    rows_a, ca = A.shape
    rows_g, cg = G.shape
    kvol = koff.shape[0] - 1
    dW = _empty((kvol, ca, cg), F32, A)
    ws_bytes = _ws_bytes(_PAIRS_WGRAD[bool(bf16)][1], n_pairs, ca, cg, kvol)
    ws = _scratch(ws_bytes, A)
    _launch_wgrad(ptr(A), rows_a, ptr(idx_a), ptr(G), rows_g, ptr(idx_g), ptr(koff), n_pairs, ca, cg, kvol, ptr(dW), ptr(ws), ws_bytes, stream(), bool(bf16))
    return dW


def _conv_shapes(feats, kernel, km, transposed):
    kvol, ca, co = kernel.shape
    n_in, n_out = (km.n_out, km.n_in) if transposed else (km.n_in, km.n_out)
    if feats.shape != (n_in, ca) or km.kvol != kvol:
        raise ValueError(f"conv3d: shape mismatch feats {tuple(feats.shape)} kernel {tuple(kernel.shape)} map ({km.kvol},{n_in}->{n_out})")
    return kvol, ca, co, n_in, n_out


def _map_sides(km, transposed):
    if transposed:
        return km.pair_out, km.pos, km.pair_in, km.pos_t
    return km.pair_in, km.pos_t, km.pair_out, km.pos


_EMPTY, _DIRECT, _OSTAT, _PAIRS = "empty", "direct", "ostat", "pairs"


def _conv_route(km, transposed, ca, co, kvol, rows, bf16, grad=False):
    if grad:
        if rows == 0 or km.n_pairs == 0:
            return _EMPTY
        return _DIRECT if (not transposed and km.fine_bijective) else _PAIRS
    if transposed and km.fine_bijective:
        return _DIRECT
    if rows == 0 or km.n_pairs == 0:
        return _EMPTY
    if not bf16 and not transposed and ostat_preferred(ca, co, kvol, rows=rows):
        return _OSTAT
    return _PAIRS


def _conv_forward(feats, kernel, km, transposed, bf16=False):
    kvol, ca, co, n_in, n_out = _conv_shapes(feats, kernel, km, transposed)
    route = _conv_route(km, transposed, ca, co, kvol, n_out, bf16)
    src, _, dst, dst_pos = _map_sides(km, transposed)
    if route == _DIRECT:
        return _spconv_direct(feats, kernel, src, dst, km.koff, km.n_pairs, n_out, co, 0, bf16=bf16)
    if route == _OSTAT:
        return _spconv_ostat(feats, kernel, km.nbr, n_out, co, 0, 0, pairs=km.n_pairs)
    return _spconv_apply(feats, kernel, src, dst_pos, km.koff, km.n_pairs, n_out, co, 0, bf16=bf16)


def _conv_backward(feats, kernel, km, transposed, grad_out, need_feats, need_kernel, bf16=False):
    kvol, ca, co = kernel.shape
    n_feats = feats.shape[0]
    g_feats = g_kernel = None
    src, src_pos, dst, _ = _map_sides(km, transposed)
    if need_feats:
        route = _conv_route(km, transposed, co, ca, kvol, n_feats, bf16, grad=True)
        if route == _EMPTY:
            g_feats = torch.zeros((n_feats, ca), dtype=F32, device=feats.device)
        elif route == _DIRECT:
            g_feats = _spconv_direct(grad_out, kernel, dst, src, km.koff, km.n_pairs, n_feats, ca, 1, bf16=bf16)
        else:
            g_feats = _spconv_apply(grad_out, kernel, dst, src_pos, km.koff, km.n_pairs, n_feats, ca, 1, bf16=bf16)
    if need_kernel:
        g_kernel = _spconv_wgrad(feats, src, grad_out, dst, km.koff, km.n_pairs, bf16=bf16)
    return g_feats, g_kernel


class _SparseConv(torch.autograd.Function):

    @staticmethod
    def forward(ctx, feats, kernel, km, transposed, bf16=False):
        feats = req(feats.contiguous(), F32, "conv3d feats", 2)
        kernel = req(kernel.contiguous(), F32, "conv3d kernel", 3)
        out = _conv_forward(feats, kernel, km, transposed, bf16)
        ctx.save_for_backward(feats, kernel)
        ctx.km, ctx.transposed, ctx.bf16 = km, transposed, bf16
        return out

    @staticmethod
    def backward(ctx, grad_out):
        feats, kernel = ctx.saved_tensors
        grad_out = req(grad_out.contiguous(), F32, "conv3d grad", 2)
        g_feats, g_kernel = _conv_backward(feats, kernel, ctx.km, ctx.transposed, grad_out, ctx.needs_input_grad[0], ctx.needs_input_grad[1], ctx.bf16)
        return g_feats, g_kernel, None, None, None


def sparse_conv(feats, kernel, km, transposed=False, bf16=False):
    return _SparseConv.apply(feats, kernel, km, transposed, bool(bf16))


def _rows_gemm(A, W, w_transposed, bias, co, bf16=False):
    L = _lib.load()
    n, ca = A.shape
    out = _empty((n, co), F32, A)
    fn = _ROWS_GEMM[bool(bf16)]
    check(getattr(L, fn)(ptr(A), n, ptr(W), int(w_transposed), ptr(bias), ca, co, ptr(out), stream()), fn)
    return out


def _rows_wgrad(A, G, bf16=False):
    L = _lib.load()
    fn, ws_fn, _ = _PAIRS_WGRAD[bool(bf16)]
    n, ca = A.shape
    cg = G.shape[1]
    dW = _empty((1, ca, cg), F32, A)
    ws_bytes = _ws_bytes(ws_fn, n, ca, cg, 1)
    ws = _scratch(ws_bytes, A)
    check(getattr(L, fn)(ptr(A), n, 0, ptr(G), n, 0, 0, n, ca, cg, 1, ptr(dW), ptr(ws), ws_bytes, stream()), fn + "(dense)")
    return dW[0]


def _rows_ok(*channels):
    return all(c >= 4 and c % 4 == 0 for c in channels)


class _RowsLinear(torch.autograd.Function):

    @staticmethod
    def forward(ctx, x, weight, bias, bf16=False):
        x = req(x.contiguous(), F32, "linear x", 2)
        weight = req(weight.contiguous(), F32, "linear weight", 2)
        co, ca = weight.shape
        if x.shape[1] != ca:
            raise ValueError("linear: shape mismatch")
        _channel_operands(x, co, "linear", optional=("bias",), bias=bias)
        ctx.save_for_backward(x, weight)
        ctx.has_bias, ctx.bf16 = bias is not None, bf16
        return _rows_gemm(x, weight, 1, bias, co, bf16)

    @staticmethod
    def backward(ctx, go):
        x, weight = ctx.saved_tensors
        go = req(go.contiguous(), F32, "linear grad", 2)
        gx = gw = gb = None
        if ctx.needs_input_grad[0]:
            gx = _rows_gemm(go, weight, 0, None, weight.shape[1], ctx.bf16)
        if ctx.needs_input_grad[1]:
            gw = _rows_wgrad(go, x, ctx.bf16)
        if ctx.has_bias and ctx.needs_input_grad[2]:
            gb = colsum(go) if go.shape[1] % 4 == 0 else go.sum(0)
        return gx, gw, gb, None


class _RowsMatmul(torch.autograd.Function):

# ... 98 lines not shown
        mean = _empty((c,), F32, x)
        invstd = _empty((c,), F32, x)
        ws_bytes = _ws_bytes("ftx_bn_workspace_bytes", n, c)
        ws = _scratch(ws_bytes, x)
        _launch_bn_fwd(ptr(x), ptr(residual), ptr(gamma), ptr(beta), ptr(running_mean), ptr(running_var), momentum, eps, n, c, relu, ptr(y), ptr(mean),
                       ptr(invstd), _stream_scratch(), ptr(ws), ws_bytes)
        ctx.save_for_backward(x, y, gamma, beta, mean, invstd)
        ctx.relu = int(relu)
        ctx.has_res = residual is not None
        ctx.remask = bool(remask)
        return y

    @staticmethod
    def backward(ctx, gy):
        x, y, gamma, beta, mean, invstd = ctx.saved_tensors
        gy = req(gy.contiguous(), F32, "bn grad", 2)
        n, c = x.shape
        gx = torch.empty_like(x)
        gres = torch.empty_like(x) if ctx.has_res else None
        ggamma = _empty((c,), F32, x)
        gbeta = _empty((c,), F32, x)
        ws_bytes = _ws_bytes("ftx_bn_workspace_bytes", n, c)
        ws = _scratch(ws_bytes, x)
        _launch_bn_bwd(ptr(gy), ptr(x), ptr(y), ptr(gamma), ptr(beta) if ctx.remask else 0, ptr(mean), ptr(invstd), n, c, ctx.relu, ptr(gx), ptr(gres),
                       ptr(ggamma), ptr(gbeta), ptr(ws), ws_bytes, _stream_scratch())
        return gx, gres, ggamma, gbeta, None, None, None, None, None, None


class _BatchNormEval(torch.autograd.Function):
    @staticmethod
    def forward(ctx, x, residual, gamma, beta, running_mean, running_var, eps, relu):
        L = _lib.load()
        x = req(x.contiguous(), F32, "bn x", 2)
        n, c = x.shape
        residual = _bn_operands(residual, gamma, beta, n, c, "bn", "parameter length != channels")
        _channel_operands(x, c, "bn", running_mean=running_mean, running_var=running_var)
        y = torch.empty_like(x)
        check(L.ftx_bn_eval_fwd(ptr(x), ptr(residual), ptr(gamma), ptr(beta), ptr(running_mean), ptr(running_var), float(eps), n, c, int(relu),
                                ptr(y), stream()), "ftx_bn_eval_fwd")
        need_gamma = ctx.needs_input_grad[2]
        ctx.save_for_backward(y, gamma, running_var, x if need_gamma else None, running_mean if need_gamma else None)
        ctx.eps, ctx.relu, ctx.has_res = float(eps), int(relu), residual is not None
        return y

    @staticmethod
    def backward(ctx, gy):
        y, gamma, running_var, x, running_mean = ctx.saved_tensors
        dy = gy * (y > 0) if ctx.relu else gy
        invstd = torch.rsqrt(running_var + ctx.eps)
        scale = gamma * invstd
        gx = dy * scale
        sums = colsum if gy.shape[1] % 4 == 0 else (lambda t: t.sum(0))
        ggamma = sums(dy * ((x - running_mean) * invstd)) if ctx.needs_input_grad[2] else None
        gbeta = sums(dy) if ctx.needs_input_grad[3] else None
        return gx, (dy if ctx.has_res else None), ggamma, gbeta, None, None, None, None


class _ConvBNTrain(torch.autograd.Function):

    @staticmethod
    def forward(ctx, feats, kernel, km, transposed, residual, gamma, beta, running_mean, running_var, momentum, eps, relu, bf16, remask):
        feats = req(feats.contiguous(), F32, "conv3d feats", 2)
        kernel = req(kernel.contiguous(), F32, "conv3d kernel", 3)
        kvol, ca, co, n_in, n_out = _conv_shapes(feats, kernel, km, transposed)
        residual = _bn_operands(residual, gamma, beta, n_out, co, "conv_bn", "BatchNorm parameter length != output channels")
        _channel_operands(feats, co, "conv_bn", optional=_RUNNING, running_mean=running_mean, running_var=running_var)
        stats = _empty((2, co), F32, feats)
        x = _empty((n_out, co), F32, feats)
        y = torch.empty_like(x)
        st = _stream_scratch()
        route = _conv_route(km, transposed, ca, co, kvol, n_out, bf16)
        src, _, dst, dst_pos = _map_sides(km, transposed)
        tmp_bytes = 0 if route in (_DIRECT, _OSTAT) else 4 * km.n_pairs * co
        if route in (_OSTAT, _PAIRS):
            nb = _ws_bytes("ftx_spconv_ostat_blocks", n_out) if route == _OSTAT else _ws_bytes("ftx_spconv_reduce_stats_blocks", n_out, co)
            tmp, part = _carve(feats, tmp_bytes, 16 * (nb + 1) * co)
            ws = ws_bytes = 0
            totals = part + 16 * nb * co
        else:
            ws_bytes = _ws_bytes("ftx_bn_workspace_bytes", n_out, co)
            tmp, ws = _carve(feats, tmp_bytes, ws_bytes)
            part = nb = totals = 0
        if route == _DIRECT:
            _launch_direct(ptr(feats), n_in, ptr(src), ptr(dst), ptr(kernel), 0, ptr(km.koff), km.n_pairs, ca, co, kvol, ptr(x), n_out, st, bf16)
        elif route == _OSTAT:
            _launch_ostat(ptr(feats), n_in, ptr(km.nbr), n_out, ptr(kernel), 0, 0, ca, co, kvol, ptr(x), part, nb, st, km.n_pairs)
        else:
            _launch_pairs(ptr(feats), n_in, ptr(src), ptr(kernel), 0, ptr(dst_pos), ptr(km.koff), km.n_pairs, ca, co, kvol, tmp, ptr(x), n_out, st, bf16,
                          part, nb)
        _launch_bn_fwd(ptr(x), ptr(residual), ptr(gamma), ptr(beta), ptr(running_mean), ptr(running_var), momentum, eps, n_out, co, relu, ptr(y),
                       stats.data_ptr(), stats.data_ptr() + 4 * co, st, ws, ws_bytes, totals)
        ctx.save_for_backward(feats, kernel, x, y, gamma, beta, stats)
        ctx.km, ctx.transposed, ctx.relu, ctx.has_res, ctx.bf16, ctx.remask = km, transposed, int(relu), residual is not None, bf16, bool(remask)
        return y

    @staticmethod
    def backward(ctx, gy):
        feats, kernel, x, y, gamma, beta, stats = ctx.saved_tensors
        km, transposed, bf16 = ctx.km, ctx.transposed, ctx.bf16
        gy = req(gy.contiguous(), F32, "conv_bn grad", 2)
        n, co = x.shape
        kvol, ca, _ = kernel.shape
        n_feats = feats.shape[0]
        need_feats, need_kernel = ctx.needs_input_grad[0], ctx.needs_input_grad[1]
        st = _stream_scratch()
        gparams = _empty((2, co), F32, x)
        gres = torch.empty_like(x) if ctx.has_res else None
        src, src_pos, dst, _ = _map_sides(km, transposed)
        route = _conv_route(km, transposed, co, ca, kvol, n_feats, bf16, grad=True) if need_feats else None
        bn_ws_bytes = _ws_bytes("ftx_bn_workspace_bytes", n, co)
        wg_bytes = _ws_bytes(_PAIRS_WGRAD[bf16][1], km.n_pairs, ca, co, kvol) if (need_kernel and km.n_pairs > 0) else 0
        bn_ws, gx, tmp, wg_ws = _carve(x, bn_ws_bytes, 4 * n * co, 4 * km.n_pairs * ca if route == _PAIRS else 0, wg_bytes)
        _launch_bn_bwd(ptr(gy), ptr(x), ptr(y), ptr(gamma), ptr(beta) if ctx.remask else 0, stats.data_ptr(), stats.data_ptr() + 4 * co, n, co, ctx.relu,
                       gx, ptr(gres), gparams.data_ptr(), gparams.data_ptr() + 4 * co, bn_ws, bn_ws_bytes, st)
        g_feats = g_kernel = None
        if need_feats:
            g_feats = _empty((n_feats, ca), F32, x)
            if route == _EMPTY:
                g_feats.zero_()
            elif route == _DIRECT:
                _launch_direct(gx, n, ptr(dst), ptr(src), ptr(kernel), 1, ptr(km.koff), km.n_pairs, co, ca, kvol, ptr(g_feats), n_feats, st, bf16)
            else:
                _launch_pairs(gx, n, ptr(dst), ptr(kernel), 1, ptr(src_pos), ptr(km.koff), km.n_pairs, co, ca, kvol, tmp, ptr(g_feats), n_feats, st, bf16)
        if need_kernel:
            g_kernel = _empty((kvol, ca, co), F32, x)
            _launch_wgrad(ptr(feats), n_feats, ptr(src), gx, n, ptr(dst), ptr(km.koff), km.n_pairs, ca, co, kvol, ptr(g_kernel), wg_ws, wg_bytes, st, bf16)
        return g_feats, g_kernel, None, None, gres, gparams[0], gparams[1], None, None, None, None, None, None, None


def conv_bn_train(feats, kernel, km, transposed, gamma, beta, running_mean, running_var, momentum=0.1, eps=1e-5, residual=None, relu=False,
                  bf16=False, remask=True):
    return _ConvBNTrain.apply(feats, kernel, km, transposed, residual, gamma, beta, running_mean, running_var, momentum, eps, relu, bool(bf16),
                              bool(remask))


def batch_norm(x, gamma, beta, running_mean, running_var, training, momentum=0.1, eps=1e-5, residual=None, relu=False, remask=True):
    if training:
        return _BatchNormTrain.apply(x, residual, gamma, beta, running_mean, running_var, momentum, eps, relu, bool(remask))
    return _BatchNormEval.apply(x, residual, gamma, beta, running_mean, running_var, eps, relu)


def spconv_reduce_bn_eval(tmp, pos, n_out, gamma, beta, running_mean, running_var, eps=1e-5, residual=None, relu=False):
    L = _lib.load()
    tmp = req(tmp, F32, "reduce_bn_eval tmp", 2)
    req(pos, I32, "reduce_bn_eval pos", 2)
    co, kvol = tmp.shape[1], pos.shape[0]
    if pos.shape[1] != n_out:
        raise ValueError("reduce_bn_eval: the position table does not match the output rows")
    for t, nm in ((gamma, "gamma"), (beta, "beta"), (running_mean, "running_mean"), (running_var, "running_var")):
        req(t, F32, "reduce_bn_eval " + nm, 1)
        if t.shape[0] != co:
            raise ValueError("reduce_bn_eval: BatchNorm parameter length != output channels")
    if residual is not None:
        residual = req(residual.contiguous(), F32, "reduce_bn_eval residual", 2)
        if residual.shape != (n_out, co):
            raise ValueError("reduce_bn_eval: residual shape mismatch")
    out = _empty((n_out, co), F32, tmp)
    _log_launch("spconv_reduce", dict(pairs=tmp.shape[0], n_out=n_out, ca=0, co=co, kvol=kvol), lambda: check(L.ftx_spconv_reduce_bn_eval(
        ptr(tmp), ptr(pos), n_out, co, kvol, ptr(residual), ptr(gamma), ptr(beta), ptr(running_mean), ptr(running_var), float(eps), int(relu), ptr(out),
        stream()), "ftx_spconv_reduce_bn_eval"))
    return out


def conv_bn_eval(feats, kernel, km, transposed, gamma, beta, running_mean, running_var, eps=1e-5, residual=None, relu=False, bf16=False):
    feats = req(feats.contiguous(), F32, "conv3d feats", 2)
    kernel = req(kernel.contiguous(), F32, "conv3d kernel", 3)
    kvol, ca, co, n_in, n_out = _conv_shapes(feats, kernel, km, transposed)
    route = _conv_route(km, transposed, ca, co, kvol, n_out, bf16)
    if route in (_PAIRS, _EMPTY) and kvol in (8, 27):
        src, _, _, dst_pos = _map_sides(km, transposed)
        L = _lib.load()
        tmp = _empty((km.n_pairs, co), F32, feats)
        gemm, kind = _PAIRS_GEMM[bool(bf16)]
        _log_launch(kind, dict(pairs=km.n_pairs, n_out=n_out, ca=ca, co=co, kvol=kvol), lambda: check(getattr(L, gemm)(
            ptr(feats), n_in, ptr(src), ptr(kernel), 0, ptr(km.koff), km.n_pairs, ca, co, kvol, ptr(tmp), stream()), gemm))
        return spconv_reduce_bn_eval(tmp, dst_pos, n_out, gamma, beta, running_mean, running_var, eps, residual=residual, relu=relu)
    with torch.no_grad():
        return batch_norm(_conv_forward(feats, kernel, km, transposed, bool(bf16)), gamma, beta, running_mean, running_var, False, eps=eps,
                          residual=residual, relu=relu)


def rows_concat(a, b):
    a, b = req(a, F32, "rows_concat a", 2), req(b, F32, "rows_concat b", 2)
    if a.shape[0] != b.shape[0]:
        raise ValueError("rows_concat: row counts differ")
    out = _empty((a.shape[0], a.shape[1] + b.shape[1]), F32, a)
    check(_lib.load().ftx_rows_concat(ptr(a), a.shape[1], ptr(b), b.shape[1], a.shape[0], ptr(out), stream()), "ftx_rows_concat")
    return out


def rows_split(x, ca):
    x = req(x, F32, "rows_split x", 2)
    n, cb = x.shape[0], x.shape[1] - int(ca)
    a, b = _empty((n, int(ca)), F32, x), _empty((n, cb), F32, x)
    check(_lib.load().ftx_rows_split(ptr(x), n, int(ca), cb, ptr(a), ptr(b), stream()), "ftx_rows_split")
    return a, b


def rows_add(a, b):
    a, b = req(a, F32, "rows_add a", 2), req(b, F32, "rows_add b", 2)
    if a.shape != b.shape:
        raise ValueError("rows_add: shapes differ")
    out = torch.empty_like(a)
    check(_lib.load().ftx_rows_add(ptr(a), ptr(b), a.shape[0], a.shape[1], ptr(out), stream()), "ftx_rows_add")
    return out


def lift_segments(img_idx, point_batch, b, gh, gw, H, W) -> Segments:
    L = _lib.load()
    req(img_idx, I64, "lift img_idx", 2)
    req(point_batch, I32, "lift point_batch", 1)
    n = img_idx.shape[0]
    cells = _empty((n,), I32, point_batch)
    check(L.ftx_lift_cells(ptr(img_idx), ptr(point_batch), n, int(b), int(gh), int(gw), int(H), int(W), ptr(cells), stream()), "ftx_lift_cells")
    return Segments(cells, int(b) * int(gh) * int(gw))


class _LiftGather(torch.autograd.Function):
    @staticmethod
    def forward(ctx, grid, img_idx, point_batch, H, W, seg):
        L = _lib.load()
        grid = req(grid.contiguous(), F32, "lift grid", 4)
        req(img_idx, I64, "lift img_idx", 2)
        req(point_batch, I32, "lift point_batch", 1)
        b, gh, gw, c = grid.shape
        n = img_idx.shape[0]
        if img_idx.shape != (n, 2) or point_batch.shape[0] != n:
            raise ValueError("lift_gather: img_idx must be (N,2), point_batch (N,)")
        out = _empty((n, c), F32, grid)
        check(L.ftx_lift_gather_fwd(ptr(grid), ptr(img_idx), ptr(point_batch), n, b, gh, gw, c, int(H), int(W), ptr(out), stream()), "ftx_lift_gather_fwd")
        ctx.save_for_backward(img_idx, point_batch)
        ctx.dims = (b, gh, gw, c, int(H), int(W))
        ctx.seg = seg
        return out

    @staticmethod
    def backward(ctx, go):
        L = _lib.load()
        img_idx, point_batch = ctx.saved_tensors
        b, gh, gw, c, H, W = ctx.dims
        go = req(go.contiguous(), F32, "lift grad", 2)
        gg = _empty((b, gh, gw, c), F32, go)
        seg = ctx.seg
        if seg is not None:
            if seg.m != b * gh * gw or seg.order.shape[0] != go.shape[0]:
                raise ValueError("lift_gather: segments do not match the grid / points")
            check(L.ftx_segment_sum(ptr(go), ptr(seg.order), ptr(seg.seg_off), go.shape[0], c, seg.m, ptr(gg), stream()), "ftx_segment_sum")
        else:
            check(L.ftx_lift_gather_bwd(ptr(go), ptr(img_idx), ptr(point_batch), go.shape[0], b, gh, gw, c, H, W, ptr(gg), stream()), "ftx_lift_gather_bwd")
        return gg, None, None, None, None, None


def lift_gather(grid, img_idx, point_batch, H, W, seg=None):
    return _LiftGather.apply(grid, img_idx, point_batch, H, W, seg)


class _ResampleNearest(torch.autograd.Function):
    @staticmethod
# ... 779 lines not shown
```

fusiontransformer_amd/native_index.py:

```python
from __future__ import annotations

import ctypes

import numpy as np
import torch

from . import _lib
from . import functional as spf
from .native_eval import MAP, MAP_KEYS, PV, PV_STRIDES, STRIDES
from .sparse import CoordinateManager, HostRead, KernelMap, PointTensor, SparseTensor

_vp = ctypes.c_void_p
_DT = {"i32": (torch.int32, 4), "i64": (torch.int64, 8), "f32": (torch.float32, 4)}

WORDS = (["a_total", "b_total", "c_total", "a_coords", "a_points", "a_uniq", "a_first", "a_skeys", "a_order"]
         + [f"{k}{l}" for l in range(5) for k in ("coords", "tkeys", "tvals", "cap")] + ["x0"]
         + [f"{k}{m}" for m in range(9) for k in ("nbr", "pos", "koff")]
         + [f"{k}{m}" for m in range(5, 9) for k in ("pos_t", "pair_in", "pair_out")]
         + [f"{k}{j}" for j in range(3) for k in ("vidx", "vcnt", "vseg", "didx", "dw", "dorder", "dseg")]
         + [f"{k}{m}" for m in range(5) for k in ("pos_t", "pair_in", "pair_out")])


class Refused(Exception):
    """The library refused the batch before launching anything (its text is the message); the caller takes the per-op path."""
# ... 58 lines not shown
    return t


def _alloc(nbytes, device):
    return torch.empty((int(nbytes),), dtype=torch.uint8, device=device)


def index_steps(x, init_res, after_res, with_backward_segments=None):
    L = _lib.load()
    if with_backward_segments is None:
        with_backward_segments = torch.is_grad_enabled()
    bwd = int(bool(with_backward_segments))
    coords = x.C
    if coords.dtype != torch.float32:
        coords = coords.float()
    coords = coords.contiguous()
    feats = x.F
    if not (torch.is_tensor(feats) and feats.is_cuda and coords.is_cuda and feats.dtype == torch.float32 and feats.dim() == 2
            and coords.dim() == 2 and coords.shape[1] == 4 and feats.shape[0] == coords.shape[0]):
        raise Refused("native index: (n, 4) coordinates and (n, c) float32 features on the GPU expected")
    feats_c = feats.contiguous()
    n, c_in = int(feats.shape[0]), int(feats.shape[1])
    dev = coords.device
    st = _lib.stream()
    ir, ar = float(init_res), float(after_res)
    if c_in < 4 or c_in % 4 or c_in > 1024:
        raise Refused("native index: the feature width must be a multiple of 4 in [4, 1024]")
    lay = layout(n, c_in)
    arena_a = _alloc(lay["a_total"], dev)
    pinned = torch.empty((16,), dtype=torch.int32, pin_memory=True)
    rc = L.ftx_spvcnn_index_levels(coords.data_ptr(), n, ir, ar, arena_a.data_ptr(), arena_a.shape[0], pinned.data_ptr(), st)
    if rc != 0:
        raise Refused(_error())
    read = _Read(pinned)
    yield "sync"
    level_off = read.values(6)
    try:
        lay = layout(n, c_in, level_off, None, bwd)
    except Refused as e:
        raise RuntimeError(f"native index: {e}") from None
    arena_b = _alloc(lay["b_total"], dev)
    pinned2 = torch.empty((16,), dtype=torch.int32, pin_memory=True)
    _lib.check(L.ftx_spvcnn_index_maps(coords.data_ptr(), n, ir, ar, feats_c.data_ptr(), c_in, _np_ptr(level_off), bwd, arena_a.data_ptr(), arena_a.shape[0],
                                       arena_b.data_ptr(), arena_b.shape[0], pinned2.data_ptr(), st), "ftx_spvcnn_index_maps")
    read = _Read(pinned2)
    yield "sync"
    pair_counts = read.values(5)
    try:
        lay = layout(n, c_in, level_off, pair_counts, bwd)
    except Refused as e:
        raise RuntimeError(f"native index: {e}") from None
    arena_c = _alloc(lay["c_total"], dev)
    rows = np.zeros(6, dtype=np.int64)
    maps = np.zeros(len(MAP_KEYS), dtype=MAP)
    pvs = np.zeros(len(PV_STRIDES), dtype=PV)
    _lib.check(L.ftx_spvcnn_index_pairs(n, c_in, _np_ptr(level_off), bwd, _np_ptr(pair_counts), arena_a.data_ptr(), arena_b.data_ptr(), arena_b.shape[0],
                                        arena_c.data_ptr(), arena_c.shape[0], _np_ptr(rows), _np_ptr(maps), _np_ptr(pvs), None, st), "ftx_spvcnn_index_pairs")
    return _structures(feats, coords, n, c_in, ir != ar, bwd, lay, level_off, pair_counts, arena_a, arena_b, arena_c, (rows, maps, pvs))


def _structures(feats, coords, n, c_in, rescaled, bwd, lay, level_off, pair_counts, A, B, C, tables):
    sizes = [int(level_off[l + 1] - level_off[l]) for l in range(5)]
    points = _view(A, lay["a_points"], "i32", n, 4)
    uniq = _view(A, lay["a_uniq"], "i64", 5 * n)
    first = _view(A, lay["a_first"], "i32", 5 * n)
    skeys = _view(A, lay["a_skeys"], "i64", 5, n)
    order = _view(A, lay["a_order"], "i32", 5, n)
    cm = CoordinateManager()
    cm.points = points
    cm.level_data = {}
    for l, s in enumerate(STRIDES):
        lo, hi = int(level_off[l]), int(level_off[l + 1])
        cm.level_data[s] = (uniq[lo:hi], first[lo:hi], l, skeys[l], order[l])
        cm.coords[s] = _view(B, lay[f"coords{l}"], "i32", sizes[l], 4)
        cap = lay[f"cap{l}"]
        cm.tables[s] = _table(_view(B, lay[f"tkeys{l}"], "i64", cap), _view(B, lay[f"tvals{l}"], "i32", cap), sizes[l], cap)
    for m, key in enumerate(MAP_KEYS):
        ks, s, stride = key
        l = STRIDES.index(s)
        sub = stride == 1
        k, n_in, n_out = (27, sizes[l], sizes[l]) if sub else (8, sizes[l], sizes[l + 1])
        n_pairs = int(pair_counts[l]) if sub else n_in
        arena = C if sub else B
        cm.kernel_maps[key] = KernelMap(_view(B, lay[f"nbr{m}"], "i32", k, n_out), _view(B, lay[f"pos{m}"], "i32", k, n_out),
                                        _view(arena, lay[f"pos_t{m}"], "i32", k, n_in), _view(arena, lay[f"pair_in{m}"], "i32", n_pairs),
                                        _view(arena, lay[f"pair_out{m}"], "i32", n_pairs), _view(B, lay[f"koff{m}"], "i32", k + 1), n_pairs, n_in, n_out,
                                        cm.coords[s * stride], fine_bijective=not sub, submanifold=sub)
    zc = _view(A, lay["a_coords"], "f32", n, 4) if rescaled else coords
    z = PointTensor(feats, zc)
    af = z.additional_features
    af["vox_seg"], af["devox_seg"] = {}, {}
    for j, s in enumerate(PV_STRIDES):
        l = STRIDES.index(s)
        af["idx_query"][s] = _view(B, lay[f"vidx{j}"], "i32", n)
        af["counts"][s] = _view(B, lay[f"vcnt{j}"], "i32", sizes[l])
        af["vox_seg"][s] = spf.Segments.from_parts(order[l], _view(B, lay[f"vseg{j}"], "i32", sizes[l] + 1), sizes[l])
        z.idx_query[s] = _view(B, lay[f"didx{j}"], "i32", n, 8)
        z.weights[s] = _view(B, lay[f"dw{j}"], "f32", n, 8)
        af["devox_seg"][s] = spf.Segments.from_parts(_view(B, lay[f"dorder{j}"], "i32", 8 * n), _view(B, lay[f"dseg{j}"], "i32", sizes[l] + 1),
                                                     sizes[l]) if bwd else None
    x0 = SparseTensor(_view(B, lay["x0"], "f32", sizes[0], c_in), cm.coords[1], 1)
    x0.cm = cm
    x0.check()
    x0.native_tables = tables
    return z, x0
```

fusiontransformer_amd/sparse.py:

```python
from __future__ import annotations

import numpy as np
import torch

from . import functional as Fn


class KernelMap:
    __slots__ = ("nbr", "pos", "pos_t", "pair_in", "pair_out", "koff", "n_pairs", "n_in", "n_out", "out_coords", "kvol", "fine_bijective", "submanifold")

    def __init__(self, nbr, pos, pos_t, pair_in, pair_out, koff, n_pairs, n_in, n_out, out_coords, fine_bijective=False, submanifold=False):
        self.nbr, self.pos, self.pos_t, self.pair_in, self.pair_out, self.koff = nbr, pos, pos_t, pair_in, pair_out, koff
        self.n_pairs, self.n_in, self.n_out, self.out_coords = n_pairs, n_in, n_out, out_coords
        self.kvol = nbr.shape[0]
        self.fine_bijective = bool(fine_bijective) and n_pairs == n_in
        self.submanifold = bool(submanifold) and n_in == n_out and self.kvol % 2 == 1


class CoordinateManager:

    def __init__(self):
        self.tables = {}
        self.coords = {}
        self.kernel_maps = {}
        self._offsets = {}
        self.points = None
        self.level_data = None

    def offsets(self, ks, stride, device):
        key = (ks, stride)
        if key not in self._offsets:
            self._offsets[key] = torch.from_numpy(Fn.kernel_offsets(ks, stride)).to(device)
        return self._offsets[key]

    def table(self, stride):
        if stride not in self.tables:
            self.tables[stride] = Fn.HashTable(Fn.sphash(self.coords[stride]))
        return self.tables[stride]

    def _materialize_level(self, stride):
        if stride in self.coords or not self.level_data or stride not in self.level_data:
            return stride in self.coords
        hashes, first = self.level_data[stride][:2]
        self.coords[stride] = Fn.level_coords(self.points, first, stride)
        if stride not in self.tables:
            self.tables[stride] = Fn.HashTable(hashes)
        return True

    def kernel_map(self, ks, cur_stride, stride) -> KernelMap:
        key = (ks, cur_stride, stride)
        km = self.kernel_maps.get(key)
        if km is not None:
            return km
        return drain(self.kernel_map_steps(ks, cur_stride, stride))

    def kernel_map_steps(self, ks, cur_stride, stride):
        key = (ks, cur_stride, stride)
        km = self.kernel_maps.get(key)
        if km is not None:
            return km
        coords = self.coords[cur_stride]
        n_in = coords.shape[0]
        table = self.table(cur_stride)
        off = self.offsets(ks, cur_stride, coords.device)
        if stride == 1:
            out_coords = coords
        else:
            new_stride = cur_stride * stride
            if new_stride not in self.coords and not self._materialize_level(new_stride):
                yield from self.downsample_steps(cur_stride, stride)
            out_coords = self.coords[new_stride]
        nbr = Fn.kernel_map_build(out_coords, off, table)
        pos, koff = Fn.kernel_map_count(nbr)
        if ks == stride and ks == 2:
            n_pairs = n_in
        else:
            pending = HostRead(koff[-1:])
            yield "sync"
            n_pairs = pending.value()
        return self._finish_map(key, nbr, pos, koff, n_pairs, n_in, out_coords)

    def _finish_map(self, key, nbr, pos, koff, n_pairs, n_in, out_coords):
        pos, pos_t, pair_in, pair_out = Fn.kernel_map_pairs(nbr, pos, n_in, n_pairs)
        ks, cur_stride, stride = key
        km = KernelMap(nbr, pos, pos_t, pair_in, pair_out, koff, n_pairs, n_in, out_coords.shape[0], out_coords,
                       fine_bijective=(ks == stride == 2), submanifold=(stride == 1 and ks % 2 == 1))
        self.kernel_maps[key] = km
        return km

    def downsample_steps(self, cur_stride, stride):
        launched = self._downsample_launch(cur_stride, stride)
        yield "sync"
        self._downsample_finish(cur_stride * stride, *launched)

    def _downsample_launch(self, cur_stride, stride):
        down = Fn.downsample_coords(self.coords[cur_stride], cur_stride * stride)
        uniq, first, cnt = Fn.unique_sorted(Fn.sphash(down))
        return down, first, HostRead(cnt)

    def _downsample_finish(self, new_stride, down, first, pending):
        n_out = pending.value()
        self.coords[new_stride] = Fn.gather_coords(down, first[:n_out].contiguous())

    def unet_levels_steps(self, strides, ks=3, down_ks=2):
        if self.level_data and all(s in self.level_data for s in strides):
            pend = []
            for s in strides:
                self._materialize_level(s)
                coords = self.coords[s]
                nbr = Fn.kernel_map_build(coords, self.offsets(ks, s, coords.device), self.table(s))
                pos, koff = Fn.kernel_map_count(nbr)
                pend.append((s, coords, nbr, pos, koff))
            pending = HostRead(torch.cat([koff[-1:] for _, _, _, _, koff in pend]))
            yield "sync"
            for (s, coords, nbr, pos, koff), n_pairs in zip(pend, pending.values()):
                self._finish_map((ks, s, 1), nbr, pos, koff, n_pairs, coords.shape[0], coords)
            for s, nxt in zip(strides[:-1], strides[1:]):
                drain(self.kernel_map_steps(down_ks, s, nxt // s))
            return
        for i, s in enumerate(strides):
            coords = self.coords[s]
            n_in = coords.shape[0]
            key = (ks, s, 1)
            nbr = Fn.kernel_map_build(coords, self.offsets(ks, s, coords.device), self.table(s))
            pos, koff = Fn.kernel_map_count(nbr)
            last = i + 1 == len(strides)
            if last:
                pending = HostRead(koff[-1:])
                yield "sync"
                self._finish_map(key, nbr, pos, koff, pending.value(), n_in, coords)
                break
            ratio = strides[i + 1] // s
            down = Fn.downsample_coords(coords, s * ratio)
            uniq, first, cnt = Fn.unique_sorted(Fn.sphash(down))
            pending = HostRead(torch.cat([koff[-1:].to(cnt.dtype), cnt]))
            yield "sync"
            n_pairs, n_out = pending.values()
            self._finish_map(key, nbr, pos, koff, n_pairs, n_in, coords)
            self.coords[s * ratio] = Fn.gather_coords(down, first[:n_out].contiguous())
            drain(self.kernel_map_steps(down_ks, s, ratio))


class HostRead:

    latest = None

    def __init__(self, dev: torch.Tensor):
        self.host = torch.empty(dev.shape, dtype=dev.dtype, pin_memory=True)
        self.host.copy_(dev, non_blocking=True)
        self.event = torch.cuda.Event()
        self.event.record()
        HostRead.latest = self

    def ready(self):
        return self.event.query()

    def values(self):
        self.event.synchronize()
        return [int(v) for v in self.host.tolist()]

    def value(self):
        return self.values()[0]


def drain(steps):
    while True:
        try:
            next(steps)
        except StopIteration as done:
# ... 120 lines not shown
```

include/ftx.h:

```cpp
#ifndef FTX_H
#define FTX_H

#include <stddef.h>
#include <stdint.h>

#ifdef __cplusplus
extern "C" {
#endif

#define FTX_OK 0
#define FTX_EINVAL -1
#define FTX_ELAUNCH -2
#define FTX_EWORKSPACE -3

int ftx_version(void);
const char *ftx_last_error(void);

size_t ftx_stream_scratch_bytes(void);
int ftx_stream_scratch_attach(void *stream, void *buffer, size_t bytes);
int ftx_stream_scratch_reset(void *stream);
int ftx_stream_scratch_release(void *stream);


int ftx_hash(const int32_t *coords, int64_t n, int64_t *out, void *stream);

int ftx_hash_kernel(const int32_t *coords, int64_t n, const int32_t *offsets, int32_t k, int64_t *out, void *stream);

int ftx_floor_coords(const float *pc, int64_t n, int32_t stride, int32_t *out, void *stream);


int64_t ftx_hashtable_capacity(int64_t n);
int ftx_hashtable_build(const int64_t *keys, int64_t n, int64_t *table_keys, int32_t *table_vals, int64_t capacity, void *stream);
int ftx_hashtable_query(const int64_t *queries, int64_t nq, const int64_t *table_keys, const int32_t *table_vals, int64_t capacity, int32_t *out, void *stream);

int ftx_count(const int32_t *idx, int64_t n, int32_t *counts, int64_t m, void *stream);

size_t ftx_unique_workspace_bytes(int64_t n);
int ftx_unique_sorted(const int64_t *keys, int64_t n, int64_t *uniq, int32_t *first_index, int32_t *n_unique, void *workspace, size_t workspace_bytes, void *stream);
int ftx_rotate_points(const float *points, int64_t n, const float *rot_host, float *out, void *stream);
int ftx_sorted_rank(const int64_t *sorted, const int32_t *n_sorted, int64_t capacity, const int64_t *queries, int64_t nq, int32_t *rank, void *stream);

int ftx_downsample_coords(const int32_t *coords, int64_t n, int32_t ratio, int32_t *out, void *stream);

int ftx_gather_coords(const int32_t *src, const int32_t *index, int64_t n, int32_t *out, void *stream);

size_t ftx_levels_workspace_bytes(int64_t n, int32_t n_levels);
int ftx_levels_unique(const int32_t *points, int64_t n, const int32_t *strides, int32_t n_levels, int64_t *uniq, int32_t *first_index, int32_t *level_off, int64_t *sorted_keys, int32_t *order, void *workspace, size_t workspace_bytes, void *stream);
int ftx_level_segments(const int64_t *sorted_keys, int64_t n, const int64_t *uniq, int64_t m, int32_t level, int32_t *seg_off, void *stream);
int ftx_level_coords(const int32_t *points, const int32_t *first_index, int64_t n, int32_t stride, int32_t *out, void *stream);


int ftx_kernel_map_build(const int32_t *out_coords, int64_t n_out, const int32_t *offsets, int32_t k, const int64_t *table_keys, const int32_t *table_vals, int64_t capacity, int32_t *nbr, void *stream);
size_t ftx_kernel_map_count_workspace_bytes(int64_t n_out, int32_t k);
int ftx_kernel_map_count(const int32_t *nbr, int64_t n_out, int32_t k, int32_t *pos, int32_t *koff, void *workspace, size_t workspace_bytes, void *stream);
int ftx_kernel_map_pairs(const int32_t *nbr, int64_t n_out, int64_t n_in, int32_t k, int32_t *pos, int32_t *pos_t, int32_t *pair_in, int32_t *pair_out, int64_t n_pairs, void *stream);

int ftx_trilinear_weights(const float *pc, const int32_t *idx, int64_t n, int32_t scale, float *weights, void *stream);


int ftx_voxelize_fwd(const float *feats, const int32_t *idx, const int32_t *counts, int64_t n, int32_t c, int64_t m, float *out, void *stream);
int ftx_voxelize_bwd(const float *grad_out, const int32_t *idx, const int32_t *counts, int64_t n, int32_t c, int64_t m, float *grad_feats, void *stream);

int ftx_devoxelize_fwd(const float *feats, const int32_t *idx, const float *weights, int64_t n, int32_t c, int64_t m, float *out, void *stream);
int ftx_devoxelize_bwd(const float *grad_out, const int32_t *idx, const float *weights, int64_t n, int32_t c, int64_t m, float *grad_feats, void *stream);

size_t ftx_segment_workspace_bytes(int64_t n, int64_t m);
int ftx_segment_build(const int32_t *keys, int64_t n, int64_t m, int32_t *order, int32_t *seg_off, void *workspace, size_t workspace_bytes, void *stream);
int ftx_voxelize_fwd_sorted(const float *feats, const int32_t *order, const int32_t *seg_off, int64_t n, int32_t c, int64_t m, float *out, void *stream);
int ftx_devoxelize_bwd_sorted(const float *grad_out, const float *weights, const int32_t *order, const int32_t *seg_off, int64_t n, int32_t c, int64_t m, float *grad_feats, void *stream);

int ftx_segment_sum(const float *src, const int32_t *order, const int32_t *seg_off, int64_t n, int32_t c, int64_t m, float *out, void *stream);


int ftx_lift_gather_fwd(const float *grid, const int64_t *img_idx, const int32_t *point_batch, int64_t n, int32_t b, int32_t gh, int32_t gw, int32_t c, int32_t H, int32_t W, float *out, void *stream);
int ftx_lift_gather_bwd(const float *grad_out, const int64_t *img_idx, const int32_t *point_batch, int64_t n, int32_t b, int32_t gh, int32_t gw, int32_t c, int32_t H, int32_t W, float *grad_grid, void *stream);

int ftx_lift_cells(const int64_t *img_idx, const int32_t *point_batch, int64_t n, int32_t b, int32_t gh, int32_t gw, int32_t H, int32_t W, int32_t *cells, void *stream);

int ftx_resample_nearest_fwd(const float *in, int32_t b, int32_t c, int32_t ih, int32_t iw, int32_t oh, int32_t ow, float *out, void *stream);
int ftx_resample_nearest_bwd(const float *grad_out, int32_t b, int32_t c, int32_t ih, int32_t iw, int32_t oh, int32_t ow, float *grad_in, void *stream);

size_t ftx_sample_down_workspace_bytes(void);
int ftx_sample_down_fwd(const float *img, int32_t b, int32_t h, int32_t w, int32_t oh, int32_t ow, const float *conv_w, const float *conv_b, const float *gamma, const float *beta, float *running_mean, float *running_var, float momentum, float eps, int32_t training, float *out, double *saved, void *workspace, size_t workspace_bytes, void *stream);
int ftx_sample_down_bwd(const float *img, const float *grad_out, int32_t b, int32_t h, int32_t w, int32_t oh, int32_t ow, const float *conv_w, const float *conv_b, const float *gamma, const double *saved, float *grad_conv_w, float *grad_conv_b, float *grad_gamma, float *grad_beta, void *workspace, size_t workspace_bytes, void *stream);

int ftx_affine_sample_fwd(const float *src, const int64_t *src_strides, int32_t b, int32_t c, int32_t ih, int32_t iw, const float *theta, int32_t oh, int32_t ow, float *out, void *stream);
size_t ftx_affine_theta_workspace_bytes(int32_t b);
int ftx_affine_sample_bwd_theta(const float *src, const int64_t *src_strides, int32_t b, int32_t c, int32_t ih, int32_t iw, const float *theta, const float *grad_out, int32_t oh, int32_t ow, float *grad_theta, void *workspace, size_t workspace_bytes, void *stream);
int ftx_affine_lift_fwd(const float *src, const int64_t *src_strides, int32_t b, int32_t c, int32_t ih, int32_t iw, const float *theta, const int64_t *img_idx, const int32_t *point_batch, int64_t n, int32_t H, int32_t W, float *out, void *stream);
int ftx_affine_lift_cells(const float *theta, const int64_t *img_idx, const int32_t *point_batch, int64_t n, int32_t b, int32_t ih, int32_t iw, int32_t H, int32_t W, int32_t *cells, void *stream);
int ftx_affine_lift_bwd(const float *src, const int64_t *src_strides, int32_t b, int32_t c, int32_t ih, int32_t iw, const float *theta, const int64_t *img_idx, const int32_t *point_batch, const float *grad_out, int64_t n, int32_t H, int32_t W, const int32_t *order, const int32_t *seg_off, float *grad_src, float *grad_theta, void *workspace, size_t workspace_bytes, void *stream);

size_t ftx_loc_conv_pool_relu_fwd_workspace_bytes(int32_t b, int32_t co, int32_t ph, int32_t pw);
int ftx_loc_conv_pool_relu_fwd(const float *x, const int64_t *x_strides, int32_t b, int32_t c, int32_t ih, int32_t iw, const float *w, const float *bias, int32_t k, int32_t co, float *out, int8_t *sel, float *mean, void *workspace, size_t workspace_bytes, void *stream);
size_t ftx_loc_conv_pool_relu_bwd_weight_workspace_bytes(int32_t b, int32_t c, int32_t ih, int32_t iw, int32_t k, int32_t co);
int ftx_loc_conv_pool_relu_bwd_weight(const float *x, const int64_t *x_strides, int32_t b, int32_t c, int32_t ih, int32_t iw, const int8_t *sel, const float *grad, const int64_t *grad_strides, int32_t k, int32_t co, float *grad_w, float *grad_bias, void *workspace, size_t workspace_bytes, void *stream);
int ftx_loc_conv_pool_relu_bwd_data(const float *w, const int8_t *sel, const float *grad, const int64_t *grad_strides, int32_t b, int32_t c, int32_t ih, int32_t iw, int32_t k, int32_t co, float *grad_x, const int64_t *grad_x_strides, void *stream);


int ftx_spconv_pairs_gemm(const float *A, int64_t rows_a, const int32_t *gather, const float *W, int32_t w_transposed, const int32_t *koff, int64_t n_pairs, int32_t ca, int32_t co, int32_t kvol, float *tmp, void *stream);

int ftx_spconv_pairs_gemm_scatter(const float *A, int64_t rows_a, const int32_t *gather, const int32_t *scatter, const float *W, int32_t w_transposed, const int32_t *koff, int64_t n_pairs, int32_t ca, int32_t co, int32_t kvol, float *out, int64_t rows_out, void *stream);

int32_t ftx_spconv_ostat_supported(int32_t ca, int32_t co, int32_t kvol, int32_t w_transposed);
int32_t ftx_spconv_ostat_blocks(int64_t n_out);
int ftx_spconv_ostat(const float *A, int64_t rows_a, const int32_t *nbr, int64_t n_out, const float *W, int32_t w_transposed, int32_t flip, int32_t ca, int32_t co, int32_t kvol, float *out, double *part, int32_t nb, void *stream);

int ftx_rows_gemm(const float *A, int64_t n, const float *W, int32_t w_transposed, const float *bias, int32_t ca, int32_t co, float *out, void *stream);
int32_t ftx_spconv_gemm_block_cols(int32_t co, int64_t n_pairs, int32_t kvol);

int ftx_spconv_reduce(const float *tmp, const int32_t *pos, int64_t n, int32_t co, int32_t kvol, float *out, void *stream);

int ftx_spconv_reduce_bn_eval(const float *tmp, const int32_t *pos, int64_t n, int32_t co, int32_t kvol, const float *residual, const float *gamma, const float *beta, const float *running_mean, const float *running_var, float eps, int32_t relu, float *out, void *stream);

int32_t ftx_spconv_reduce_stats_blocks(int64_t n, int32_t co);
int ftx_spconv_reduce_stats(const float *tmp, const int32_t *pos, int64_t n, int32_t co, int32_t kvol, float *out, double *part, int32_t nb, void *stream);

size_t ftx_spconv_pairs_wgrad_workspace_bytes(int64_t n_pairs, int32_t ca, int32_t cg, int32_t kvol);
int ftx_spconv_pairs_wgrad(const float *A, int64_t rows_a, const int32_t *idx_a, const float *G, int64_t rows_g, const int32_t *idx_g, const int32_t *koff, int64_t n_pairs, int32_t ca, int32_t cg, int32_t kvol, float *dW, void *workspace, size_t workspace_bytes, void *stream);
int32_t ftx_spconv_wgrad_resident_blocks(int32_t ca, int32_t cg);
int32_t ftx_spconv_wgrad_table_blocks(int32_t mi, int32_t wmg, int32_t ni, int32_t wng);

int ftx_spconv_pairs_gemm_bf16(const float *A, int64_t rows_a, const int32_t *gather, const float *W, int32_t w_transposed, const int32_t *koff, int64_t n_pairs, int32_t ca, int32_t co, int32_t kvol, float *tmp, void *stream);
int ftx_spconv_pairs_gemm_scatter_bf16(const float *A, int64_t rows_a, const int32_t *gather, const int32_t *scatter, const float *W, int32_t w_transposed, const int32_t *koff, int64_t n_pairs, int32_t ca, int32_t co, int32_t kvol, float *out, int64_t rows_out, void *stream);
int ftx_rows_gemm_bf16(const float *A, int64_t n, const float *W, int32_t w_transposed, const float *bias, int32_t ca, int32_t co, float *out, void *stream);
size_t ftx_spconv_pairs_wgrad_bf16_workspace_bytes(int64_t n_pairs, int32_t ca, int32_t cg, int32_t kvol);
int ftx_spconv_pairs_wgrad_bf16(const float *A, int64_t rows_a, const int32_t *idx_a, const float *G, int64_t rows_g, const int32_t *idx_g, const int32_t *koff, int64_t n_pairs, int32_t ca, int32_t cg, int32_t kvol, float *dW, void *workspace, size_t workspace_bytes, void *stream);
int32_t ftx_spconv_gemm_bf16_block_cols(int32_t co, int64_t n_pairs, int32_t kvol);
int32_t ftx_spconv_wgrad_bf16_table_blocks(int32_t mi, int32_t wmg, int32_t ni, int32_t wng);


size_t ftx_bn_workspace_bytes(int64_t n, int32_t c);
int ftx_bn_train_fwd(const float *x, const float *residual, const float *gamma, const float *beta, float *running_mean, float *running_var, float momentum, float eps, int64_t n, int32_t c, int32_t relu, float *y, float *save_mean, float *save_invstd, void *workspace, size_t workspace_bytes, void *stream);
int ftx_bn_train_fwd_totals(const float *x, const float *residual, const float *gamma, const float *beta, float *running_mean, float *running_var, float momentum, float eps, int64_t n, int32_t c, int32_t relu, float *y, float *save_mean, float *save_invstd, const double *totals, void *stream);

int ftx_bn_eval_fwd(const float *x, const float *residual, const float *gamma, const float *beta, const float *running_mean, const float *running_var, float eps, int64_t n, int32_t c, int32_t relu, float *y, void *stream);
int ftx_bn_train_bwd(const float *grad_y, const float *x, const float *y, const float *gamma, const float *beta, const float *save_mean, const float *save_invstd, int64_t n, int32_t c, int32_t relu, float *grad_x, float *grad_residual, float *grad_gamma, float *grad_beta, void *workspace, size_t workspace_bytes, void *stream);

int32_t ftx_adam_chunk_elements(void);
int32_t ftx_adam_tensor_bytes(void);
int ftx_adam_step(const void *table, const int32_t *chunk_tensor, const int64_t *chunk_offset, int32_t n_chunks, double beta1, double beta2, float eps, float weight_decay, void *stream);

int ftx_add_layernorm_fwd(const float *x, const float *y, const float *y_bias, const float *gamma, const float *beta, float eps, int64_t rows, int32_t c, float *s_out, float *h_out, float *mean, float *rstd, void *stream);
size_t ftx_layernorm_bwd_workspace_bytes(int64_t rows, int32_t c);
int ftx_add_layernorm_bwd(const float *grad_h, const float *grad_s, const float *s, const float *gamma, const float *mean, const float *rstd, int64_t rows, int32_t c, int32_t with_y_bias, float *grad_x, float *grad_params, void *workspace, size_t workspace_bytes, void *stream);

size_t ftx_colsum_workspace_bytes(int64_t rows, int32_t cols);
int ftx_colsum(const float *x, int64_t rows, int32_t cols, float *out, void *workspace, size_t workspace_bytes, void *stream);


int ftx_attn_fwd(const float *qkv, int32_t b, int32_t t, int32_t h, int32_t d, float scale, float *out, float *lse, void *stream);
size_t ftx_attn_bwd_workspace_bytes(int32_t b, int32_t t, int32_t h);
int ftx_attn_bwd(const float *qkv, const float *out, const float *grad_out, const float *lse, int32_t b, int32_t t, int32_t h, int32_t d, float scale, float *grad_qkv, void *workspace, size_t workspace_bytes, void *stream);
int ftx_attn_fwd_tiled(const float *qkv, int32_t b, int32_t t, int32_t h, int32_t d, float scale, float *out, float *lse, int32_t qw, int32_t split, void *stream);
int ftx_attn_bwd_tiled(const float *qkv, const float *out, const float *grad_out, const float *lse, int32_t b, int32_t t, int32_t h, int32_t d, float scale, float *grad_qkv, void *workspace, size_t workspace_bytes, int32_t qw, int32_t split, void *stream);
int ftx_attn_fwd_bf16(const float *qkv, int32_t b, int32_t t, int32_t h, int32_t d, float scale, float *out, float *lse, int32_t qw, int32_t split, void *stream);
int ftx_attn_bwd_bf16(const float *qkv, const float *out, const float *grad_out, const float *lse, int32_t b, int32_t t, int32_t h, int32_t d, float scale, float *grad_qkv, void *workspace, size_t workspace_bytes, int32_t qw, int32_t split, void *stream);

#define FTX_EPI_NONE 0
#define FTX_EPI_BIAS 1
#define FTX_EPI_BIAS_GELU 2
#define FTX_EPI_DGELU 3
int ftx_dense_gemm_bf16(const float *A, const float *W, int32_t w_kn, const float *bias, const float *pre_in, int64_t m, int32_t n, int32_t k, int32_t epilogue, float *out, float *pre_out, void *stream);
size_t ftx_dense_wgrad_bf16_workspace_bytes(int64_t m, int32_t n, int32_t k);
int ftx_dense_wgrad_bf16(const float *dY, const float *X, int64_t m, int32_t n, int32_t k, float *dW, void *workspace, size_t workspace_bytes, void *stream);
int ftx_dense_bf16_tile(int32_t form, int64_t m, int32_t n, int32_t k, int32_t *tile_m_host, int32_t *tile_n_host, int32_t *split_host);

int ftx_dense_gemm_split(const float *A, const float *W, int32_t w_kn, const float *bias, const float *pre_in, int64_t m, int32_t n, int32_t k, int32_t epilogue, float *out, float *pre_out, void *stream);
size_t ftx_dense_wgrad_split_workspace_bytes(int64_t m, int32_t n, int32_t k);
int ftx_dense_wgrad_split(const float *dY, const float *X, int64_t m, int32_t n, int32_t k, float *dW, void *workspace, size_t workspace_bytes, void *stream);
int ftx_dense_split_tile(int32_t form, int64_t m, int32_t n, int32_t k, int32_t *tile_m_host, int32_t *tile_n_host, int32_t *split_host);

size_t ftx_fusion_loss_workspace_bytes(void);
int ftx_fusion_loss_mix(const float *lidar_logit, const float *img_logit, const float *lidar_logit2, const float *img_logit2, const int64_t *label, const float *class_weights, float ce_scale, float lambda_xm, int64_t n, int32_t c, int32_t ignore_index, float *losses, float *grad_lidar, float *grad_img, float *grad_lidar2, float *grad_img2, int64_t *conf3d, int64_t *conf2d, void *workspace, size_t workspace_bytes, void *stream);
int ftx_fusion_loss(const float *lidar_logit, const float *img_logit, const float *lidar_logit2, const float *img_logit2, const int64_t *label, const float *class_weights, float lambda_xm, int64_t n, int32_t c, int32_t ignore_index, float *losses, float *grad_lidar, float *grad_img, float *grad_lidar2, float *grad_img2, int64_t *conf3d, int64_t *conf2d, void *workspace, size_t workspace_bytes, void *stream);

size_t ftx_seg_loss_workspace_bytes(void);
int ftx_seg_loss(const float *logit, const int64_t *label, const float *class_weights, int64_t n, int32_t c, int32_t ignore_index, float *loss, float *grad, int64_t *conf, void *workspace, size_t workspace_bytes, void *stream);

int ftx_eval_scatter_back(const float *logits3d, const float *logits2d, int64_t n_rows, int32_t num_classes, const int64_t *inverse, const int32_t *gt, int64_t m, const int32_t *class_labels, int32_t *pred3d, int32_t *pred2d, int32_t *pred_ens, int64_t *conf3d, int64_t *conf2d, int64_t *conf_ens, int32_t *bad_flag, void *stream);

int ftx_project_points(const float *points, int64_t n, const float *proj_matrix, int32_t width, int32_t height, uint8_t *keep, float *rowcol, void *stream);

#define FTX_JITTER_BRIGHTNESS 0
#define FTX_JITTER_CONTRAST 1
// ... 71 lines not shown
```

Measured before the change: 151.6.

## Precompute per-block tile table for sparse-conv pair GEMMs and overlap epilogue with MFMA

Builds a tile table once per kernel map that gives each GEMM block its kernel offset, first pair and count. Blocks then read their tile directly instead of scanning koff and syncing at start. For NT=2 the last K-chunk is unrolled so each 32-column tile is stored while MFMAs for the next tile run, and launch bounds request higher occupancy. This costs extra memory and a build kernel per map, and the tighter launch bounds may raise register pressure or cause spills.

```diff
diff --git a/fusiontransformer_amd/_lib.py b/fusiontransformer_amd/_lib.py
--- a/fusiontransformer_amd/_lib.py
+++ b/fusiontransformer_amd/_lib.py
@@ -69,6 +69,11 @@
     "ftx_loc_conv_pool_relu_bwd_data": (C.c_int, [_vp, _vp, _vp, _vp, _i32, _i32, _i32, _i32, _i32, _i32, _vp, _vp, _vp]),
     "ftx_spconv_pairs_gemm": (C.c_int, [_vp, _i64, _vp, _vp, _i32, _vp, _i64, _i32, _i32, _i32, _vp, _vp]),
     "ftx_spconv_pairs_gemm_scatter": (C.c_int, [_vp, _i64, _vp, _vp, _vp, _i32, _vp, _i64, _i32, _i32, _i32, _vp, _i64, _vp]),
+    "ftx_spconv_tile_table_entries": (_i64, [_i64, _i32, _i32]),
+    "ftx_spconv_tile_table": (C.c_int, [_vp, _i32, _i32, _i64, _vp, _vp]),
+    "ftx_spconv_tile_table_host": (C.c_int, [_vp, _i32, _i32, _i64, _vp]),
+    "ftx_spconv_pairs_gemm_tiles": (C.c_int, [_vp, _i64, _vp, _vp, _i32, _vp, _i64, _i32, _i32, _i32, _vp, _vp]),
+    "ftx_spconv_pairs_gemm_scatter_tiles": (C.c_int, [_vp, _i64, _vp, _vp, _vp, _i32, _vp, _i64, _i32, _i32, _i32, _vp, _i64, _vp]),
     "ftx_spconv_ostat_supported": (_i32, [_i32, _i32, _i32, _i32]),
     "ftx_spconv_ostat_blocks": (_i32, [_i64]),
     "ftx_spconv_ostat": (C.c_int, [_vp, _i64, _vp, _i64, _vp, _i32, _i32, _i32, _i32, _i32, _vp, _vp, _i32, _vp]),
diff --git a/fusiontransformer_amd/csrc/ftx_spconv.hip b/fusiontransformer_amd/csrc/ftx_spconv.hip
--- a/fusiontransformer_amd/csrc/ftx_spconv.hip
+++ b/fusiontransformer_amd/csrc/ftx_spconv.hip
@@ -79,11 +79,12 @@
 
 constexpr int AS_STRIDE = 36;
 
-template <int NT>
-__global__ __launch_bounds__(256) void pairs_gemm_kernel(const float *__restrict__ A, int64_t rows_a, const int32_t *__restrict__ gather,
+template <int NT, bool TABLE>
+__global__ __launch_bounds__(256, NT == 2 ? 4 : 1) void pairs_gemm_kernel(const float *__restrict__ A, int64_t rows_a, const int32_t *__restrict__ gather,
                                                          const float *__restrict__ W, int w_transposed, const int32_t *__restrict__ koff,
                                                          int ca, int co, int kvol, float *__restrict__ tmp, const float *__restrict__ bias,
-                                                         int64_t n_dense, const int32_t *__restrict__ scatter, int64_t rows_out) {
+                                                         int64_t n_dense, const int32_t *__restrict__ scatter, int64_t rows_out,
+                                                         const int32_t *__restrict__ tiles, int64_t n_pairs) {
   constexpr int BN = 32 * NT;
   constexpr int BS_STRIDE = AS_STRIDE;
   constexpr int A_PASSES = kPairAPasses;
@@ -94,11 +95,17 @@
   __shared__ int s_tile[3];
 
   const int tid = threadIdx.x;
-  gemm_tile_scan(koff, kvol, n_dense, gather == nullptr, s_tile);
-  __syncthreads();
-  const int k = s_tile[0];
-  if (k < 0) return;
-  const int p0 = s_tile[1], cnt = s_tile[2];
+  int k, p0, cnt;
+  if constexpr (TABLE) {
+    if (!gemm_tile_lookup(tiles, kvol, n_pairs, k, p0, cnt)) return;
+  } else {
+    gemm_tile_scan(koff, kvol, n_dense, gather == nullptr, s_tile);
+    __syncthreads();
+    k = s_tile[0];
+    if (k < 0) return;
+    p0 = s_tile[1];
+    cnt = s_tile[2];
+  }
 
   const int wave = tid >> 6, lane = tid & 63;
   const int half = lane >> 5, l31 = lane & 31;
@@ -175,13 +182,9 @@
     }
   };
 
-  load_chunk(0);
-  for (int c0 = 0; c0 < ca; c0 += kPairBK) {
-    store_chunk();
-    __syncthreads();
-    if (c0 + kPairBK < ca) load_chunk(c0 + kPairBK);
-    const float *arow_p = &As[(wave * 32 + l31) * AS_STRIDE + 4 * half];
-    const float *brow_p = &Bs[l31 * BS_STRIDE + 4 * half];
+  const float *arow_p = &As[(wave * 32 + l31) * AS_STRIDE + 4 * half];
+  const float *brow_p = &Bs[l31 * BS_STRIDE + 4 * half];
+  auto mfma_chunk = [&]() {
     float af[2][4], bf[2][NT][4];
     auto load_frag = [&](int buf, int t) {
       float4 a = *(const float4 *)(arow_p + 8 * t);
@@ -201,9 +204,53 @@
 #pragma unroll
         for (int j = 0; j < NT; ++j) acc[j] = __builtin_amdgcn_mfma_f32_32x32x2f32(bf[t & 1][j][s], af[t & 1][s], acc[j], 0, 0, 0);
     }
+  };
+
+  load_chunk(0);
+  if constexpr (NT == 1) {
+    for (int c0 = 0; c0 < ca; c0 += kPairBK) {
+      store_chunk();
+      __syncthreads();
+      if (c0 + kPairBK < ca) load_chunk(c0 + kPairBK);
+      mfma_chunk();
+      __syncthreads();
+    }
+    pair_gemm_epilogue<NT>(acc, p0, cnt, n0, gather, rows_a, scatter, rows_out, bias, co, tmp);
+  } else {
+    int c0 = 0;
+    for (; c0 + kPairBK < ca; c0 += kPairBK) {
+      store_chunk();
+      __syncthreads();
+      load_chunk(c0 + kPairBK);
+      mfma_chunk();
+      __syncthreads();
+    }
+    store_chunk();
     __syncthreads();
-  }
-  pair_gemm_epilogue<NT>(acc, p0, cnt, n0, gather, rows_a, scatter, rows_out, bias, co, tmp);
+    const PairEpilogueRow er = pair_epilogue_row(p0, cnt, gather, rows_a, scatter, rows_out, co, tmp);
+    const bool nfull = n0 + 32 * NT <= co;
+    constexpr int TS = kPairBK / 8;
+    float4 a4[TS], b4[2];
+#pragma unroll
+    for (int t = 0; t < TS; ++t) a4[t] = *(const float4 *)(arow_p + 8 * t);
+    b4[0] = *(const float4 *)brow_p;
+#pragma unroll
+    for (int j = 0; j < NT; ++j) {
+#pragma unroll
+      for (int t = 0; t < TS; ++t) {
+        const int u = j * TS + t;
+        if (u + 1 < NT * TS) b4[(u + 1) & 1] = *(const float4 *)(brow_p + ((u + 1) / TS) * 32 * BS_STRIDE + 8 * ((u + 1) % TS));
+        const float4 a = a4[t], b = b4[u & 1];
+        acc[j] = __builtin_amdgcn_mfma_f32_32x32x2f32(b.x, a.x, acc[j], 0, 0, 0);
+        acc[j] = __builtin_amdgcn_mfma_f32_32x32x2f32(b.y, a.y, acc[j], 0, 0, 0);
+        acc[j] = __builtin_amdgcn_mfma_f32_32x32x2f32(b.z, a.z, acc[j], 0, 0, 0);
+        acc[j] = __builtin_amdgcn_mfma_f32_32x32x2f32(b.w, a.w, acc[j], 0, 0, 0);
+        __builtin_amdgcn_sched_barrier(0);
+      }
+      pair_epilogue_tile(acc[j], j, er, n0, nfull, bias, co);
+      __builtin_amdgcn_sched_barrier(0);
+    }
+  }
 }
 
 #include "ftx_lastblock.h"
@@ -519,8 +566,12 @@
   static constexpr int wgrad_step = 2 * WG_BR;
   template <int NT>
   static void gemm(dim3 grid, hipStream_t st, const PairsGemmArgs &a) {
-    pairs_gemm_kernel<NT><<<grid, 256, 0, st>>>(a.A, a.rows_a, a.gather, a.W, a.w_transposed, a.koff, a.ca, a.co, a.kvol, a.out, a.bias, a.n_dense,
-                                                a.scatter, a.rows_out);
+    if (a.tiles)
+      pairs_gemm_kernel<NT, true><<<grid, 256, 0, st>>>(a.A, a.rows_a, a.gather, a.W, a.w_transposed, a.koff, a.ca, a.co, a.kvol, a.out, a.bias,
+                                                        a.n_dense, a.scatter, a.rows_out, a.tiles, a.n_pairs);
+    else
+      pairs_gemm_kernel<NT, false><<<grid, 256, 0, st>>>(a.A, a.rows_a, a.gather, a.W, a.w_transposed, a.koff, a.ca, a.co, a.kvol, a.out, a.bias,
+                                                         a.n_dense, a.scatter, a.rows_out, nullptr, 0);
   }
   template <int MI, int NI, int WMG, int WNG>
   static void wgrad(dim3 grid, hipStream_t st, const PairsWgradArgs &a) {
@@ -533,13 +584,64 @@
 
 extern "C" int ftx_spconv_pairs_gemm(const float *A, int64_t rows_a, const int32_t *gather, const float *W, int32_t w_transposed,
                                      const int32_t *koff, int64_t n_pairs, int32_t ca, int32_t co, int32_t kvol, float *tmp, void *stream) {
-  return spconv_pairs_entry<SpconvF32>(false, A, rows_a, gather, nullptr, W, w_transposed, koff, n_pairs, ca, co, kvol, tmp, 0, stream);
+  return spconv_pairs_entry<SpconvF32>(false, A, rows_a, gather, nullptr, W, w_transposed, koff, nullptr, n_pairs, ca, co, kvol, tmp, 0, stream);
 }
 
 extern "C" int ftx_spconv_pairs_gemm_scatter(const float *A, int64_t rows_a, const int32_t *gather, const int32_t *scatter, const float *W,
                                              int32_t w_transposed, const int32_t *koff, int64_t n_pairs, int32_t ca, int32_t co, int32_t kvol,
                                              float *out, int64_t rows_out, void *stream) {
-  return spconv_pairs_entry<SpconvF32>(true, A, rows_a, gather, scatter, W, w_transposed, koff, n_pairs, ca, co, kvol, out, rows_out, stream);
+  return spconv_pairs_entry<SpconvF32>(true, A, rows_a, gather, scatter, W, w_transposed, koff, nullptr, n_pairs, ca, co, kvol, out, rows_out, stream);
+}
+
+__global__ __launch_bounds__(256) void tile_table_kernel(const int32_t *__restrict__ koff, int kvol, int tile, int64_t n_entries,
+                                                         int32_t *__restrict__ table) {
+  const int64_t b = (int64_t)blockIdx.x * 256 + threadIdx.x;
+  if (b >= n_entries) return;
+  int32_t e[3];
+  pair_tile_entry(koff, kvol, tile, b, e);
+  table[3 * b] = e[0];
+  table[3 * b + 1] = e[1];
+  table[3 * b + 2] = e[2];
+}
+
+extern "C" int64_t ftx_spconv_tile_table_entries(int64_t n_pairs, int32_t kvol, int32_t tile) {
+  if (n_pairs < 0 || kvol < 1 || tile < 1) return 0;
+  return spconv_tile_table_entries(n_pairs, kvol, tile);
+}
+
+extern "C" int ftx_spconv_tile_table(const int32_t *koff, int32_t kvol, int32_t tile, int64_t n_pairs, int32_t *table, void *stream) {
+  FTX_REQUIRE(n_pairs >= 0 && n_pairs < 0x7fffffff && kvol >= 1 && kvol <= 64 && tile >= 1, "ftx_spconv_tile_table: bad size");
+  FTX_REQUIRE(koff && table, "ftx_spconv_tile_table: null pointer");
+  const int64_t n = spconv_tile_table_entries(n_pairs, kvol, tile);
+  tile_table_kernel<<<(unsigned)ceil_div(n, 256), 256, 0, (hipStream_t)stream>>>(koff, kvol, tile, n, table);
+  return check_launch("ftx_spconv_tile_table");
+}
+
+extern "C" int ftx_spconv_tile_table_host(const int32_t *koff, int32_t kvol, int32_t tile, int64_t n_pairs, int32_t *table) {
+  FTX_REQUIRE(n_pairs >= 0 && n_pairs < 0x7fffffff && kvol >= 1 && kvol <= 64 && tile >= 1, "ftx_spconv_tile_table_host: bad size");
+  FTX_REQUIRE(koff && table, "ftx_spconv_tile_table_host: null pointer");
+  const int64_t n = spconv_tile_table_entries(n_pairs, kvol, tile);
+  for (int64_t b = 0; b < n; ++b) {
+    int32_t e[3];
+    pair_tile_entry(koff, kvol, tile, b, e);
+    table[3 * b] = e[0];
+    table[3 * b + 1] = e[1];
+    table[3 * b + 2] = e[2];
+  }
+  return FTX_OK;
+}
+
+extern "C" int ftx_spconv_pairs_gemm_tiles(const float *A, int64_t rows_a, const int32_t *gather, const float *W, int32_t w_transposed,
+                                           const int32_t *tiles, int64_t n_pairs, int32_t ca, int32_t co, int32_t kvol, float *tmp, void *stream) {
+  FTX_REQUIRE(tiles || n_pairs <= 0, "ftx_spconv_pairs_gemm_tiles: null tile table");
+  return spconv_pairs_entry<SpconvF32>(false, A, rows_a, gather, nullptr, W, w_transposed, nullptr, tiles, n_pairs, ca, co, kvol, tmp, 0, stream);
+}
+
+extern "C" int ftx_spconv_pairs_gemm_scatter_tiles(const float *A, int64_t rows_a, const int32_t *gather, const int32_t *scatter, const float *W,
+                                                   int32_t w_transposed, const int32_t *tiles, int64_t n_pairs, int32_t ca, int32_t co,
+                                                   int32_t kvol, float *out, int64_t rows_out, void *stream) {
+  FTX_REQUIRE(tiles || n_pairs <= 0, "ftx_spconv_pairs_gemm_scatter_tiles: null tile table");
+  return spconv_pairs_entry<SpconvF32>(true, A, rows_a, gather, scatter, W, w_transposed, nullptr, tiles, n_pairs, ca, co, kvol, out, rows_out, stream);
 }
 
 extern "C" int ftx_rows_gemm(const float *A, int64_t n, const float *W, int32_t w_transposed, const float *bias, int32_t ca, int32_t co,
diff --git a/fusiontransformer_amd/csrc/ftx_spconv_bf16.hip b/fusiontransformer_amd/csrc/ftx_spconv_bf16.hip
--- a/fusiontransformer_amd/csrc/ftx_spconv_bf16.hip
+++ b/fusiontransformer_amd/csrc/ftx_spconv_bf16.hip
@@ -294,13 +294,13 @@
 
 extern "C" int ftx_spconv_pairs_gemm_bf16(const float *A, int64_t rows_a, const int32_t *gather, const float *W, int32_t w_transposed,
                                           const int32_t *koff, int64_t n_pairs, int32_t ca, int32_t co, int32_t kvol, float *tmp, void *stream) {
-  return spconv_pairs_entry<SpconvBf16>(false, A, rows_a, gather, nullptr, W, w_transposed, koff, n_pairs, ca, co, kvol, tmp, 0, stream);
+  return spconv_pairs_entry<SpconvBf16>(false, A, rows_a, gather, nullptr, W, w_transposed, koff, nullptr, n_pairs, ca, co, kvol, tmp, 0, stream);
 }
 
 extern "C" int ftx_spconv_pairs_gemm_scatter_bf16(const float *A, int64_t rows_a, const int32_t *gather, const int32_t *scatter, const float *W,
                                                   int32_t w_transposed, const int32_t *koff, int64_t n_pairs, int32_t ca, int32_t co, int32_t kvol,
                                                   float *out, int64_t rows_out, void *stream) {
-  return spconv_pairs_entry<SpconvBf16>(true, A, rows_a, gather, scatter, W, w_transposed, koff, n_pairs, ca, co, kvol, out, rows_out, stream);
+  return spconv_pairs_entry<SpconvBf16>(true, A, rows_a, gather, scatter, W, w_transposed, koff, nullptr, n_pairs, ca, co, kvol, out, rows_out, stream);
 }
 
 extern "C" int ftx_rows_gemm_bf16(const float *A, int64_t n, const float *W, int32_t w_transposed, const float *bias, int32_t ca, int32_t co,
diff --git a/fusiontransformer_amd/csrc/ftx_spconv_common.h b/fusiontransformer_amd/csrc/ftx_spconv_common.h
--- a/fusiontransformer_amd/csrc/ftx_spconv_common.h
+++ b/fusiontransformer_amd/csrc/ftx_spconv_common.h
@@ -51,6 +51,31 @@
   }
 }
 
+__host__ __device__ inline void pair_tile_entry(const int32_t *koff, int kvol, int tile, int64_t b, int32_t (&e)[3]) {
+  e[0] = e[1] = e[2] = -1;
+  int64_t excl = 0;
+  for (int q = 0; q < kvol; ++q) {
+    const int c = koff[q + 1] - koff[q];
+    const int nt = (c + tile - 1) / tile;
+    if (b < excl + nt) {
+      const int t = (int)(b - excl), left = c - t * tile;
+      e[0] = q;
+      e[1] = koff[q] + t * tile;
+      e[2] = left > tile ? tile : left;
+      return;
+    }
+    excl += nt;
+  }
+}
+
+__device__ __forceinline__ bool gemm_tile_lookup(const int32_t *__restrict__ tiles, int kvol, int64_t n_pairs, int &k, int &p0, int &cnt) {
+  const int32_t *e = tiles + 3 * (int64_t)blockIdx.x;
+  k = __builtin_amdgcn_readfirstlane(e[0]);
+  p0 = __builtin_amdgcn_readfirstlane(e[1]);
+  cnt = __builtin_amdgcn_readfirstlane(e[2]);
+  return k >= 0 && k < kvol && p0 >= 0 && cnt >= 1 && cnt <= kPairTile && (int64_t)p0 + cnt <= n_pairs;
+}
+
 __device__ __forceinline__ void pair_gather_rows(const int32_t *__restrict__ gather, int p0, int cnt, int64_t rows_a, int32_t (&src)[kPairAPasses]) {
   const int arow = threadIdx.x >> 3;
 #pragma unroll
@@ -63,41 +88,52 @@
   }
 }
 
+struct PairEpilogueRow {
+  float *dst;
+  bool zero;
+};
+__device__ __forceinline__ PairEpilogueRow pair_epilogue_row(int p0, int cnt, const int32_t *__restrict__ gather, int64_t rows_a,
+                                                             const int32_t *__restrict__ scatter, int64_t rows_out, int co, float *__restrict__ out) {
+  const int wave = threadIdx.x >> 6, l31 = threadIdx.x & 31;
+  const int row = wave * 32 + l31;
+  int64_t drow = row < cnt ? p0 + row : -1;
+  PairEpilogueRow r = {nullptr, false};
+  if (gather != nullptr && drow >= 0) {
+    const int32_t sidx = gather[drow];
+    r.zero = sidx < 0 || sidx >= rows_a;
+  }
+  if (scatter != nullptr && drow >= 0) {
+    drow = scatter[drow];
+    if (drow >= rows_out) drow = -1;
+  }
+  if (drow >= 0) r.dst = out + drow * co;
+  return r;
+}
+__device__ __forceinline__ void pair_epilogue_tile(const f32x16 &acc, int j, const PairEpilogueRow &r, int n0, bool nfull, const float *__restrict__ bias, int co) {
+  if (r.dst == nullptr) return;
+  const int half = (threadIdx.x & 63) >> 5;
+#pragma unroll
+  for (int q = 0; q < 4; ++q) {
+    const int col = n0 + j * 32 + 8 * q + 4 * half;
+    if (nfull || col < co) {
+      float4 v = make_float4(acc[4 * q], acc[4 * q + 1], acc[4 * q + 2], acc[4 * q + 3]);
+      if (r.zero) v = make_float4(0.f, 0.f, 0.f, 0.f);
+      if (bias) {
+        const float4 bv = *(const float4 *)&bias[col];
+        v.x += bv.x; v.y += bv.y; v.z += bv.z; v.w += bv.w;
+      }
+      *(float4 *)&r.dst[col] = v;
+    }
+  }
+}
 template <int NT>
 __device__ __forceinline__ void pair_gemm_epilogue(const f32x16 (&acc)[NT], int p0, int cnt, int n0, const int32_t *__restrict__ gather, int64_t rows_a,
                                           const int32_t *__restrict__ scatter, int64_t rows_out, const float *__restrict__ bias, int co,
                                           float *__restrict__ out) {
-  const int wave = threadIdx.x >> 6, lane = threadIdx.x & 63;
-  const int half = lane >> 5, l31 = lane & 31;
+  const PairEpilogueRow r = pair_epilogue_row(p0, cnt, gather, rows_a, scatter, rows_out, co, out);
   const bool nfull = n0 + 32 * NT <= co;
-  const int row = wave * 32 + l31;
-  int64_t drow = row < cnt ? p0 + row : -1;
-  bool zero = false;
-  if (gather != nullptr && drow >= 0) {
-    const int32_t sidx = gather[drow];
-    zero = sidx < 0 || sidx >= rows_a;
-  }
-  if (scatter != nullptr && drow >= 0) {
-    drow = scatter[drow];
-    if (drow >= rows_out) drow = -1;
-  }
-  if (drow < 0) return;
-  float *dst = out + drow * co;
-#pragma unroll
-  for (int j = 0; j < NT; ++j)
-#pragma unroll
-    for (int q = 0; q < 4; ++q) {
-      const int col = n0 + j * 32 + 8 * q + 4 * half;
-      if (nfull || col < co) {
-        float4 v = make_float4(acc[j][4 * q], acc[j][4 * q + 1], acc[j][4 * q + 2], acc[j][4 * q + 3]);
-        if (zero) v = make_float4(0.f, 0.f, 0.f, 0.f);
-        if (bias) {
-          const float4 bv = *(const float4 *)&bias[col];
-          v.x += bv.x; v.y += bv.y; v.z += bv.z; v.w += bv.w;
-        }
-        *(float4 *)&dst[col] = v;
-      }
-    }
+#pragma unroll
+  for (int j = 0; j < NT; ++j) pair_epilogue_tile(acc[j], j, r, n0, nfull, bias, co);
 }
 
 __device__ __forceinline__ void wgrad_stage_indices(const int32_t *__restrict__ idx_a, int64_t rows_a, const int32_t *__restrict__ idx_g, int64_t rows_g,
@@ -234,7 +270,11 @@
   int64_t n_dense;
   const int32_t *scatter;
   int64_t rows_out;
+  const int32_t *tiles;
+  int64_t n_pairs;
 };
+
+inline int64_t spconv_tile_table_entries(int64_t n_pairs, int kvol, int tile) { return ceil_div(n_pairs, tile) + kvol; }
 
 inline int spconv_gemm_nt(int co, int64_t row_tiles) {
   int nt = co >= 128 ? 4 : (co + 31) / 32;
@@ -262,15 +302,16 @@
 
 template <class F>
 int spconv_pairs_entry(bool scattered, const float *A, int64_t rows_a, const int32_t *gather, const int32_t *scatter, const float *W,
-                       int32_t w_transposed, const int32_t *koff, int64_t n_pairs, int32_t ca, int32_t co, int32_t kvol, float *out, int64_t rows_out,
+                       int32_t w_transposed, const int32_t *koff, const int32_t *tiles, int64_t n_pairs, int32_t ca, int32_t co, int32_t kvol, float *out, int64_t rows_out,
                        void *stream) {
   const char *me = scattered ? F::scatter_name : F::pairs_name;
   FTX_REQUIRE(n_pairs >= 0 && rows_a >= 0 && rows_out >= 0 && kvol >= 1 && kvol <= 64, "%s: bad size", me);
   FTX_REQUIRE(ca >= 4 && ca % 4 == 0 && co >= 4 && co % 4 == 0, "%s: channels must be multiples of 4 (ca=%d co=%d)", me, ca, co);
   if (n_pairs == 0) return FTX_OK;
-  FTX_REQUIRE(A && gather && (scatter || !scattered) && W && koff && out && rows_a >= 1, "%s: null pointer or empty operand", me);
-  const PairsGemmArgs a = {A, rows_a, gather, W, w_transposed, koff, ca, co, kvol, out, nullptr, 0, scatter, rows_out};
-  spconv_launch_gemm<F>(ceil_div(n_pairs, kPairTile) + kvol, (hipStream_t)stream, a);
+  FTX_REQUIRE(A && gather && (scatter || !scattered) && W && (koff || tiles) && out && rows_a >= 1, "%s: null pointer or empty operand", me);
+  FTX_REQUIRE(n_pairs < 0x7fffffff, "%s: too many pairs", me);
+  const PairsGemmArgs a = {A, rows_a, gather, W, w_transposed, koff, ca, co, kvol, out, nullptr, 0, scatter, rows_out, tiles, n_pairs};
+  spconv_launch_gemm<F>(spconv_tile_table_entries(n_pairs, kvol, kPairTile), (hipStream_t)stream, a);
   return check_launch(me);
 }
 
@@ -282,7 +323,7 @@
   FTX_REQUIRE(ca >= 4 && ca % 4 == 0 && co >= 4 && co % 4 == 0, "%s: channels must be multiples of 4 (ca=%d co=%d)", me, ca, co);
   if (n == 0) return FTX_OK;
   FTX_REQUIRE(A && W && out, "%s: null pointer", me);
-  const PairsGemmArgs a = {A, n, nullptr, W, w_transposed, nullptr, ca, co, 1, out, bias, n, nullptr, 0};
+  const PairsGemmArgs a = {A, n, nullptr, W, w_transposed, nullptr, ca, co, 1, out, bias, n, nullptr, 0, nullptr, 0};
   spconv_launch_gemm<F>(ceil_div(n, kPairTile), (hipStream_t)stream, a);
   return check_launch(me);
 }
diff --git a/fusiontransformer_amd/functional.py b/fusiontransformer_amd/functional.py
--- a/fusiontransformer_amd/functional.py
+++ b/fusiontransformer_amd/functional.py
@@ -274,6 +274,18 @@
     return pos, pos_t, pair_in, pair_out
 
 
+PAIR_TILE = 128
+
+
+def spconv_tile_table(koff: torch.Tensor, n_pairs: int) -> torch.Tensor:
+    L = _lib.load()
+    req(koff, I32, "spconv_tile_table koff", 1)
+    kvol = koff.shape[0] - 1
+    table = _empty((int(L.ftx_spconv_tile_table_entries(int(n_pairs), kvol, PAIR_TILE)), 3), I32, koff)
+    check(L.ftx_spconv_tile_table(ptr(koff), kvol, PAIR_TILE, int(n_pairs), ptr(table), stream()), "ftx_spconv_tile_table")
+    return table
+
+
 def calc_ti_weights(pc: torch.Tensor, idx_query: torch.Tensor, scale: int = 1) -> torch.Tensor:
     L = _lib.load()
     req(pc, F32, "calc_ti_weights pc", 2)
@@ -409,15 +421,18 @@
 
 _PAIRS_GEMM = {False: ("ftx_spconv_pairs_gemm", "spconv_pairs_gemm"), True: ("ftx_spconv_pairs_gemm_bf16", "spconv_pairs_gemm_bf16")}
 _PAIRS_GEMM_SCATTER = {False: "ftx_spconv_pairs_gemm_scatter", True: "ftx_spconv_pairs_gemm_scatter_bf16"}
+_PAIRS_GEMM_TILES, _PAIRS_GEMM_SCATTER_TILES = "ftx_spconv_pairs_gemm_tiles", "ftx_spconv_pairs_gemm_scatter_tiles"
 _PAIRS_WGRAD = {False: ("ftx_spconv_pairs_wgrad", "ftx_spconv_pairs_wgrad_workspace_bytes", "spconv_pairs_wgrad"),
                 True: ("ftx_spconv_pairs_wgrad_bf16", "ftx_spconv_pairs_wgrad_bf16_workspace_bytes", "spconv_pairs_wgrad_bf16")}
 _ROWS_GEMM = {False: "ftx_rows_gemm", True: "ftx_rows_gemm_bf16"}
 
 
-def _launch_pairs(a, rows_a, gather, w, w_transposed, pos, koff, n_pairs, ca, co, kvol, tmp, out, n_out, st, bf16, part=0, nb=0):
+def _launch_pairs(a, rows_a, gather, w, w_transposed, pos, koff, n_pairs, ca, co, kvol, tmp, out, n_out, st, bf16, part=0, nb=0, tiles=0):
     L = _lib.load()
     gemm, kind = _PAIRS_GEMM[bf16]
     meta = dict(pairs=n_pairs, n_out=n_out, ca=ca, co=co, kvol=kvol)
+    if tiles and not bf16:
+        gemm, koff = _PAIRS_GEMM_TILES, tiles
     _log_launch(kind, meta, lambda: check(getattr(L, gemm)(a, rows_a, gather, w, w_transposed, koff, n_pairs, ca, co, kvol, tmp, st), gemm))
     if part:
         _log_launch("spconv_reduce", meta, lambda: check(L.ftx_spconv_reduce_stats(tmp, pos, n_out, co, kvol, out, part, nb, st), "ftx_spconv_reduce_stats"))
@@ -425,9 +440,11 @@
         _log_launch("spconv_reduce", meta, lambda: check(L.ftx_spconv_reduce(tmp, pos, n_out, co, kvol, out, st), "ftx_spconv_reduce"))
 
 
-def _launch_direct(a, rows_a, gather, scatter, w, w_transposed, koff, n_pairs, ca, co, kvol, out, n_out, st, bf16):
+def _launch_direct(a, rows_a, gather, scatter, w, w_transposed, koff, n_pairs, ca, co, kvol, out, n_out, st, bf16, tiles=0):
     L = _lib.load()
     gemm = _PAIRS_GEMM_SCATTER[bf16]
+    if tiles and not bf16:
+        gemm, koff = _PAIRS_GEMM_SCATTER_TILES, tiles
     _log_launch(_PAIRS_GEMM[bf16][1], dict(pairs=n_pairs, n_out=n_out, ca=ca, co=co, kvol=kvol, direct=True), lambda: check(getattr(L, gemm)(
         a, rows_a, gather, scatter, w, w_transposed, koff, n_pairs, ca, co, kvol, out, n_out, st), gemm))
 
@@ -461,22 +478,22 @@
         L.ftx_bn_train_bwd(gy, x, y, gamma, beta, mean, invstd, n, c, int(relu), gx, gres, ggamma, gbeta, ws, ws_bytes, st), "ftx_bn_train_bwd"))
 
 
-def _spconv_apply(A, W, gather, pos, koff, n_pairs, n_rows_out, co, w_transposed, bf16=False):
+def _spconv_apply(A, W, gather, pos, koff, n_pairs, n_rows_out, co, w_transposed, bf16=False, tiles=None):
     rows_a, ca = A.shape
     tmp = _empty((n_pairs, co), F32, A)
     out = _empty((n_rows_out, co), F32, A)
     _launch_pairs(ptr(A), rows_a, ptr(gather), ptr(W), int(w_transposed), ptr(pos), ptr(koff), n_pairs, ca, co, koff.shape[0] - 1, ptr(tmp), ptr(out),
-                  n_rows_out, stream(), bool(bf16))
+                  n_rows_out, stream(), bool(bf16), tiles=ptr(tiles))
     return out
 
 
-def _spconv_direct(A, W, gather, scatter, koff, n_pairs, n_rows_out, co, w_transposed, bf16=False):
+def _spconv_direct(A, W, gather, scatter, koff, n_pairs, n_rows_out, co, w_transposed, bf16=False, tiles=None):
     rows_a, ca = A.shape
     if n_pairs != n_rows_out:
         raise ValueError("direct sparse conv: the pair list must cover every destination row exactly once")
     out = _empty((n_rows_out, co), F32, A)
     _launch_direct(ptr(A), rows_a, ptr(gather), ptr(scatter), ptr(W), int(w_transposed), ptr(koff), n_pairs, ca, co, koff.shape[0] - 1, ptr(out),
-                   n_rows_out, stream(), bool(bf16))
+                   n_rows_out, stream(), bool(bf16), tiles=ptr(tiles))
     return out
 
 
@@ -530,6 +547,10 @@
     if transposed:
         return km.pair_out, km.pos, km.pair_in, km.pos_t
     return km.pair_in, km.pos_t, km.pair_out, km.pos
+
+
+def _map_tiles(km):
+    return getattr(km, "tiles", None)
 
 
 _EMPTY, _DIRECT, _OSTAT, _PAIRS = "empty", "direct", "ostat", "pairs"
@@ -554,10 +575,10 @@
     route = _conv_route(km, transposed, ca, co, kvol, n_out, bf16)
     src, _, dst, dst_pos = _map_sides(km, transposed)
     if route == _DIRECT:
-        return _spconv_direct(feats, kernel, src, dst, km.koff, km.n_pairs, n_out, co, 0, bf16=bf16)
+        return _spconv_direct(feats, kernel, src, dst, km.koff, km.n_pairs, n_out, co, 0, bf16=bf16, tiles=_map_tiles(km))
     if route == _OSTAT:
         return _spconv_ostat(feats, kernel, km.nbr, n_out, co, 0, 0, pairs=km.n_pairs)
-    return _spconv_apply(feats, kernel, src, dst_pos, km.koff, km.n_pairs, n_out, co, 0, bf16=bf16)
+    return _spconv_apply(feats, kernel, src, dst_pos, km.koff, km.n_pairs, n_out, co, 0, bf16=bf16, tiles=_map_tiles(km))
 
 
 def _conv_backward(feats, kernel, km, transposed, grad_out, need_feats, need_kernel, bf16=False):
@@ -570,9 +591,9 @@
         if route == _EMPTY:
             g_feats = torch.zeros((n_feats, ca), dtype=F32, device=feats.device)
         elif route == _DIRECT:
-            g_feats = _spconv_direct(grad_out, kernel, dst, src, km.koff, km.n_pairs, n_feats, ca, 1, bf16=bf16)
+            g_feats = _spconv_direct(grad_out, kernel, dst, src, km.koff, km.n_pairs, n_feats, ca, 1, bf16=bf16, tiles=_map_tiles(km))
         else:
-            g_feats = _spconv_apply(grad_out, kernel, dst, src_pos, km.koff, km.n_pairs, n_feats, ca, 1, bf16=bf16)
+            g_feats = _spconv_apply(grad_out, kernel, dst, src_pos, km.koff, km.n_pairs, n_feats, ca, 1, bf16=bf16, tiles=_map_tiles(km))
     if need_kernel:
         g_kernel = _spconv_wgrad(feats, src, grad_out, dst, km.koff, km.n_pairs, bf16=bf16)
     return g_feats, g_kernel
@@ -837,12 +858,12 @@
             tmp, ws = _carve(feats, tmp_bytes, ws_bytes)
             part = nb = totals = 0
         if route == _DIRECT:
-            _launch_direct(ptr(feats), n_in, ptr(src), ptr(dst), ptr(kernel), 0, ptr(km.koff), km.n_pairs, ca, co, kvol, ptr(x), n_out, st, bf16)
+            _launch_direct(ptr(feats), n_in, ptr(src), ptr(dst), ptr(kernel), 0, ptr(km.koff), km.n_pairs, ca, co, kvol, ptr(x), n_out, st, bf16, ptr(_map_tiles(km)))
         elif route == _OSTAT:
             _launch_ostat(ptr(feats), n_in, ptr(km.nbr), n_out, ptr(kernel), 0, 0, ca, co, kvol, ptr(x), part, nb, st, km.n_pairs)
         else:
             _launch_pairs(ptr(feats), n_in, ptr(src), ptr(kernel), 0, ptr(dst_pos), ptr(km.koff), km.n_pairs, ca, co, kvol, tmp, ptr(x), n_out, st, bf16,
-                          part, nb)
+                          part, nb, ptr(_map_tiles(km)))
         _launch_bn_fwd(ptr(x), ptr(residual), ptr(gamma), ptr(beta), ptr(running_mean), ptr(running_var), momentum, eps, n_out, co, relu, ptr(y),
                        stats.data_ptr(), stats.data_ptr() + 4 * co, st, ws, ws_bytes, totals)
         ctx.save_for_backward(feats, kernel, x, y, gamma, beta, stats)
@@ -874,9 +895,9 @@
             if route == _EMPTY:
                 g_feats.zero_()
             elif route == _DIRECT:
-                _launch_direct(gx, n, ptr(dst), ptr(src), ptr(kernel), 1, ptr(km.koff), km.n_pairs, co, ca, kvol, ptr(g_feats), n_feats, st, bf16)
+                _launch_direct(gx, n, ptr(dst), ptr(src), ptr(kernel), 1, ptr(km.koff), km.n_pairs, co, ca, kvol, ptr(g_feats), n_feats, st, bf16, ptr(_map_tiles(km)))
             else:
-                _launch_pairs(gx, n, ptr(dst), ptr(kernel), 1, ptr(src_pos), ptr(km.koff), km.n_pairs, co, ca, kvol, tmp, ptr(g_feats), n_feats, st, bf16)
+                _launch_pairs(gx, n, ptr(dst), ptr(kernel), 1, ptr(src_pos), ptr(km.koff), km.n_pairs, co, ca, kvol, tmp, ptr(g_feats), n_feats, st, bf16, tiles=ptr(_map_tiles(km)))
         if need_kernel:
             g_kernel = _empty((kvol, ca, co), F32, x)
             _launch_wgrad(ptr(feats), n_feats, ptr(src), gx, n, ptr(dst), ptr(km.koff), km.n_pairs, ca, co, kvol, ptr(g_kernel), wg_ws, wg_bytes, st, bf16)
@@ -927,8 +948,11 @@
         L = _lib.load()
         tmp = _empty((km.n_pairs, co), F32, feats)
         gemm, kind = _PAIRS_GEMM[bool(bf16)]
+        koff = ptr(km.koff)
+        if _map_tiles(km) is not None and not bf16:
+            gemm, koff = _PAIRS_GEMM_TILES, ptr(_map_tiles(km))
         _log_launch(kind, dict(pairs=km.n_pairs, n_out=n_out, ca=ca, co=co, kvol=kvol), lambda: check(getattr(L, gemm)(
-            ptr(feats), n_in, ptr(src), ptr(kernel), 0, ptr(km.koff), km.n_pairs, ca, co, kvol, ptr(tmp), stream()), gemm))
+            ptr(feats), n_in, ptr(src), ptr(kernel), 0, koff, km.n_pairs, ca, co, kvol, ptr(tmp), stream()), gemm))
         return spconv_reduce_bn_eval(tmp, dst_pos, n_out, gamma, beta, running_mean, running_var, eps, residual=residual, relu=relu)
     with torch.no_grad():
         return batch_norm(_conv_forward(feats, kernel, km, transposed, bool(bf16)), gamma, beta, running_mean, running_var, False, eps=eps,
diff --git a/fusiontransformer_amd/native_index.py b/fusiontransformer_amd/native_index.py
--- a/fusiontransformer_amd/native_index.py
+++ b/fusiontransformer_amd/native_index.py
@@ -164,10 +164,12 @@
         k, n_in, n_out = (27, sizes[l], sizes[l]) if sub else (8, sizes[l], sizes[l + 1])
         n_pairs = int(pair_counts[l]) if sub else n_in
         arena = C if sub else B
+        koff = _view(B, lay[f"koff{m}"], "i32", k + 1)
         cm.kernel_maps[key] = KernelMap(_view(B, lay[f"nbr{m}"], "i32", k, n_out), _view(B, lay[f"pos{m}"], "i32", k, n_out),
                                         _view(arena, lay[f"pos_t{m}"], "i32", k, n_in), _view(arena, lay[f"pair_in{m}"], "i32", n_pairs),
-                                        _view(arena, lay[f"pair_out{m}"], "i32", n_pairs), _view(B, lay[f"koff{m}"], "i32", k + 1), n_pairs, n_in, n_out,
-                                        cm.coords[s * stride], fine_bijective=not sub, submanifold=sub)
+                                        _view(arena, lay[f"pair_out{m}"], "i32", n_pairs), koff, n_pairs, n_in, n_out,
+                                        cm.coords[s * stride], fine_bijective=not sub, submanifold=sub,
+                                        tiles=spf.spconv_tile_table(koff, n_pairs) if n_pairs > 0 else None)
     zc = _view(A, lay["a_coords"], "f32", n, 4) if rescaled else coords
     z = PointTensor(feats, zc)
     af = z.additional_features
diff --git a/fusiontransformer_amd/sparse.py b/fusiontransformer_amd/sparse.py
--- a/fusiontransformer_amd/sparse.py
+++ b/fusiontransformer_amd/sparse.py
@@ -7,10 +7,11 @@
 
 
 class KernelMap:
-    __slots__ = ("nbr", "pos", "pos_t", "pair_in", "pair_out", "koff", "n_pairs", "n_in", "n_out", "out_coords", "kvol", "fine_bijective", "submanifold")
-
-    def __init__(self, nbr, pos, pos_t, pair_in, pair_out, koff, n_pairs, n_in, n_out, out_coords, fine_bijective=False, submanifold=False):
+    __slots__ = ("nbr", "pos", "pos_t", "pair_in", "pair_out", "koff", "n_pairs", "n_in", "n_out", "out_coords", "kvol", "fine_bijective", "submanifold", "tiles")
+
+    def __init__(self, nbr, pos, pos_t, pair_in, pair_out, koff, n_pairs, n_in, n_out, out_coords, fine_bijective=False, submanifold=False, tiles=None):
         self.nbr, self.pos, self.pos_t, self.pair_in, self.pair_out, self.koff = nbr, pos, pos_t, pair_in, pair_out, koff
+        self.tiles = tiles
         self.n_pairs, self.n_in, self.n_out, self.out_coords = n_pairs, n_in, n_out, out_coords
         self.kvol = nbr.shape[0]
         self.fine_bijective = bool(fine_bijective) and n_pairs == n_in
@@ -84,7 +85,8 @@
         pos, pos_t, pair_in, pair_out = Fn.kernel_map_pairs(nbr, pos, n_in, n_pairs)
         ks, cur_stride, stride = key
         km = KernelMap(nbr, pos, pos_t, pair_in, pair_out, koff, n_pairs, n_in, out_coords.shape[0], out_coords,
-                       fine_bijective=(ks == stride == 2), submanifold=(stride == 1 and ks % 2 == 1))
+                       fine_bijective=(ks == stride == 2), submanifold=(stride == 1 and ks % 2 == 1),
+                       tiles=Fn.spconv_tile_table(koff, n_pairs) if n_pairs > 0 else None)
         self.kernel_maps[key] = km
         return km
 
diff --git a/include/ftx.h b/include/ftx.h
--- a/include/ftx.h
+++ b/include/ftx.h
@@ -101,6 +101,13 @@
 int ftx_spconv_pairs_gemm(const float *A, int64_t rows_a, const int32_t *gather, const float *W, int32_t w_transposed, const int32_t *koff, int64_t n_pairs, int32_t ca, int32_t co, int32_t kvol, float *tmp, void *stream);
 
 int ftx_spconv_pairs_gemm_scatter(const float *A, int64_t rows_a, const int32_t *gather, const int32_t *scatter, const float *W, int32_t w_transposed, const int32_t *koff, int64_t n_pairs, int32_t ca, int32_t co, int32_t kvol, float *out, int64_t rows_out, void *stream);
+
+int64_t ftx_spconv_tile_table_entries(int64_t n_pairs, int32_t kvol, int32_t tile);
+int ftx_spconv_tile_table(const int32_t *koff, int32_t kvol, int32_t tile, int64_t n_pairs, int32_t *table, void *stream);
+int ftx_spconv_tile_table_host(const int32_t *koff, int32_t kvol, int32_t tile, int64_t n_pairs, int32_t *table);
+
+int ftx_spconv_pairs_gemm_tiles(const float *A, int64_t rows_a, const int32_t *gather, const float *W, int32_t w_transposed, const int32_t *tiles, int64_t n_pairs, int32_t ca, int32_t co, int32_t kvol, float *tmp, void *stream);
+int ftx_spconv_pairs_gemm_scatter_tiles(const float *A, int64_t rows_a, const int32_t *gather, const int32_t *scatter, const float *W, int32_t w_transposed, const int32_t *tiles, int64_t n_pairs, int32_t ca, int32_t co, int32_t kvol, float *out, int64_t rows_out, void *stream);
 
 int32_t ftx_spconv_ostat_supported(int32_t ca, int32_t co, int32_t kvol, int32_t w_transposed);
 int32_t ftx_spconv_ostat_blocks(int64_t n_out);
```

Result: slower. 149.2 (-1.6%).
